# yangye1098/Speech-Denoising-Diffusion-Model-2

Measured on AMD Instinct MI355X. Metric: denoised audio sec/sec, 1000-step UNetModified2 @16kHz, higher is better.
Workload: dtype bf16; 1 GPU; UNetModified2 config_unet.json, linear 1e-6..1e-3, T=1000, 16x16448-sample chunks per GPU, condition_in; model=UNetModified2, global_batch=16, seq_len=16448, parallelism=dp1, lane_rows=16

## Files before the change

### include/sddm_hip.h

```cpp
#ifndef SDDM_HIP_H
#define SDDM_HIP_H
#include <stdint.h>

#ifdef __cplusplus
extern "C" {
#endif

#define SDDM_ABI_VERSION 1

enum sddm_status {
  SDDM_OK = 0,
  SDDM_ERR_NOT_IMPLEMENTED = 1,
  SDDM_ERR_INVALID_ARG = 2,
  SDDM_ERR_SHAPE = 3,
  SDDM_ERR_HIP = 4,
  SDDM_ERR_STATE = 5
};

enum sddm_dtype { SDDM_F32 = 0, SDDM_BF16 = 1, SDDM_F16 = 2 };

enum sddm_transition {
  SDDM_TR_ORIGINAL = 0,
  SDDM_TR_SR3 = 1,
  SDDM_TR_SUPPORTIVE = 2,
  SDDM_TR_CONDITIONAL = 3
};

typedef struct sddm_ctx sddm_ctx;

int sddm_abi_version(void);
const char* sddm_last_error(void);

int sddm_create(int device, int compute_dtype, sddm_ctx** out);
void sddm_destroy(sddm_ctx* ctx);

int sddm_configure(sddm_ctx* ctx, const char* json);

int sddm_load_param(sddm_ctx* ctx, const char* key, const void* host_ptr, const int64_t* shape,
                    int ndim, int src_dtype);

int sddm_missing_params(sddm_ctx* ctx, int64_t* n_missing);

int sddm_sample(sddm_ctx* ctx, const float* cond, int64_t B, int64_t N, uint64_t seed,
                int64_t row_offset, float* out, void* stream);

int sddm_sample_noise(sddm_ctx* ctx, const float* cond, int64_t B, int64_t N, const float* noise, float* out,
                      void* stream);

int sddm_sample_continuous(sddm_ctx* ctx, const float* cond, int64_t B, int64_t N, uint64_t seed,
                           int64_t row_offset, float* out, float* record, int sample_inter, void* stream);

int sddm_network_forward(sddm_ctx* ctx, const float* cond, const float* x_t,
                         const float* noise_level, int64_t B, int64_t N, float* eps_out,
                         void* stream);

int sddm_transition(sddm_ctx* ctx, int mode, const float* x_t, const float* eps,
                    const float* cond, int t, int64_t B, int64_t N, uint64_t seed,
                    int64_t row_offset, float* out, void* stream);

int sddm_q_sample(sddm_ctx* ctx, int mode, const float* x0, const float* y, const float* noise,
                  const int64_t* t, const float* r, int64_t B, int64_t N, float* x_t,
                  float* combined, float* s_out, float* level_out, void* stream);

int sddm_set_conv_tuning(sddm_ctx* ctx, const char* json);

int sddm_log_spectrogram(const float* audio, int64_t B, int64_t N, int n_fft, int hop,
                         const float* window, const float* fb, int n_out, float* out, void* stream);

int sddm_initial_state(sddm_ctx* ctx, int mode, const float* cond, int64_t B, int64_t N,
                       uint64_t seed, int64_t row_offset, float* out, void* stream);

int sddm_schedule(const char* schedule, int n_timestep, double linear_start, double linear_end,
                  float* out);

int sddm_profile_enable(sddm_ctx* ctx, int enable);
int sddm_profile_read(sddm_ctx* ctx, const char* kernel_class, double* avg_ms, int64_t* launches,
                      double* bytes_per_launch, double* flops_per_launch);
int sddm_profile_ops(sddm_ctx* ctx, char* buf, int64_t buflen);

#ifdef __cplusplus
}
#endif
#endif
```

### speech-denoising-diffusion-model-2_amd/csrc/conv_strip_impl.h

```cpp
#pragma once
#include <type_traits>

#ifndef SDDM_ABL_STRIP
#define SDDM_ABL_STRIP 0
#endif
#ifndef SDDM_STRIP_WLD
#define SDDM_STRIP_WLD 1
#endif
#ifndef SDDM_STRIP_WREG
#define SDDM_STRIP_WREG 1
#endif

#include "conv_common.h"
#include "conv_tile_cfg.h"
#include "kernels.h"

namespace sddm {

static constexpr ConvShape kStripShapes[] = {
    {-1, 0, 1, 1, 1, 1, 0, 0, 0, 0, 0, 0, 0, 0, 0, 0, 0},
    {32, 0, 16, 128, 256, 128, 32, 0, 32, 0, 0, 0, 1, 0, 256, 16, 0},
    {32, 0, 16, 128, 256, 128, 32, 0, 32, 0, 0, 1, 1, 0, 256, 16, 0},
    {64, 0, 8, 64, 128, 64, 32, 0, 64, 0, 0, 0, 1, 0, 256, 8, 0},
    {32, 0, 16, 64, 128, 64, 64, 0, 64, 32, 0, 2, 1, 0, 256, 16, 0},
    {32, 0, 16, 64, 128, 64, 64, 0, 64, 0, 0, 0, 0, 1, 256, 16, 0},
    {32, 0, 8, 64, 128, 64, 32, 0, 32, 64, 64, 2, 1, 0, 256, 8, 0},
    {32, 0, 8, 64, 128, 64, 32, 32, 32, 0, 0, 0, 1, 0, 256, 8, 0},
    {32, 0, 8, 64, 128, 64, 32, 0, 32, 32, 32, 2, 1, 0, 256, 8, 0},
    {32, 0, 16, 128, 256, 128, 32, 0, 32, 0, 0, 0, 0, 1, 256, 16, 0},
    {32, 0, 16, 128, 256, 128, 32, 32, 32, 0, 0, 0, 1, 0, 256, 16, 0},
    {32, 0, 16, 128, 256, 128, 32, 0, 32, 32, 32, 2, 1, 0, 256, 16, 0},
    {32, 0, 64, 128, 512, 128, 32, 0, 32, 0, 0, 0, 1, 0, 256, 64, 1},
    {32, 0, 64, 128, 512, 128, 32, 0, 32, 0, 0, 1, 1, 0, 256, 64, 1},
    {64, 0, 64, 64, 256, 64, 32, 0, 64, 0, 0, 0, 1, 0, 256, 64, 1},
    {32, 0, 128, 64, 256, 64, 64, 0, 64, 32, 0, 2, 1, 0, 256, 128, 1},
    {32, 0, 128, 64, 256, 64, 64, 0, 64, 0, 0, 0, 0, 1, 256, 128, 1},
    {32, 0, 64, 64, 256, 64, 32, 0, 32, 64, 64, 2, 1, 0, 256, 64, 1},
    {32, 0, 64, 64, 256, 64, 32, 32, 32, 0, 0, 0, 1, 0, 256, 64, 1},
    {32, 0, 64, 64, 256, 64, 32, 0, 32, 32, 32, 2, 1, 0, 256, 64, 1},
    {32, 0, 64, 128, 512, 128, 32, 0, 32, 0, 0, 0, 0, 1, 256, 64, 1},
    {32, 0, 64, 128, 512, 128, 32, 32, 32, 0, 0, 0, 1, 0, 256, 64, 1},
    {32, 0, 64, 128, 512, 128, 32, 0, 32, 32, 32, 2, 1, 0, 256, 64, 1},
};
static constexpr int kNStripShapes = (int)(sizeof(kStripShapes) / sizeof(kStripShapes[0]));

__host__ inline bool strip_shape_matches(const ConvShape& c, int nblk, int mpi, int SR, const ConvArgs& a) {
  return c.cfg == nblk && c.nw == mpi && c.nb == SR && c.Ho == a.Ho && c.Wo == a.Wo && c.CA == a.CA && c.CB == a.CB &&
         c.Cout == a.Cout && c.RCA == a.RCA && c.RCB == a.RCB && c.res == a.res_mode &&
         c.gn == (a.gamma != nullptr ? 1 : 0) && c.up == (a.upsample ? 1 : 0) && a.n_tiles == c.Ho / SR &&
         a.Hi == (c.up ? c.Ho / 2 : c.Ho) && a.Wi == (c.up ? c.Wo / 2 : c.Wo);
}

template <typename T, int FC, int W, int CIN, int MPI, int RES, bool GN, int SH>
__global__ __launch_bounds__(MPI * 2) void conv_strip_kernel(ConvArgs a, int SR_) {
  constexpr ConvShape SC = kStripShapes[SH];
  constexpr bool CS = SH > 0;
  SDDM_SHAPE_GEO(SC, CS, false, a)
  const int SR = CS ? SC.nb : SR_;
  (void)gTR; (void)gTW; (void)gTX; (void)gRes; (void)gGN; (void)gWo;
  constexpr int NT = MPI * 2;
  constexpr int NWV = NT / 64;
  constexpr int ES = (int)sizeof(T);
  constexpr int NBLK = 16 * FC, FP = 2;
  constexpr int TR = MPI / W, R = 2 * TR + 2;
  constexpr int UPP = CIN * ES / 16;
  constexpr int UPL = ES / 2;
  constexpr int VE = 16 / ES;
  constexpr int PL = ((W + 2) * 16 + 255) / 256 * 256;
  constexpr int SLOT = UPP * PL;
  constexpr int NCK = CIN / 32;
  constexpr int WPL = NBLK * 16;
  constexpr int WPLANES = NCK * 9 * 4 * UPL;
  constexpr int PB = 64 / UPP;
  constexpr int NU = TR * W * UPP;
  constexpr int UPT = NU / NT;
  constexpr int IU = ((TR + 2) * W * UPP + NT - 1) / NT;
  constexpr int RCKM = 4;
  static_assert(UPP >= 1 && UPP <= 64 && (64 % UPP) == 0, "channel units must divide a wave");
  static_assert(NU % NT == 0, "prefetch must split evenly");
  typedef T vec4 __attribute__((ext_vector_type(4)));
  extern __shared__ __attribute__((aligned(16))) char smem[];

  const int tid = threadIdx.x, lane = tid & 63, wave = tid >> 6, g = lane >> 4;
  int strip, b, zb;
  xcd_block<SDDM_XCD_ZIN != 0>(gNT, gCout / NBLK, strip, b, zb);
  const int n0 = zb * NBLK;
  const int H = gHo;
  const int RC = gRCA + gRCB;
  const int rck = RES == 2 ? RC / 32 : 0;
  constexpr bool gn = GN;

  char* ring = smem;
  char* wl = ring + R * SLOT;
  char* rw = wl + WPLANES * WPL;
  const int RPLANES = rck * 32 * ES / 16;
  float* gsc = (float*)(rw + RPLANES * WPL);
  float* red = gsc + 2 * CIN;

  const int y0 = strip * SR;
  const int iters = SR / TR;
  SDDM_STAMP(a, 0);
  GNLoad gl;
  const GNFuse gf{a.gstA, a.gtilesA, a.gntileA, a.gstB, a.gtilesB, a.gntileB, a.gamma, a.beta, a.groups, a.eps};
  gl.issue(gf, b, gCA, gCB, gn, a.bias);
  const T* srcAb = (const T*)a.srcA + (size_t)b * gHi * gWi * gCA;
  const T* srcBb = gCB ? (const T*)a.srcB + (size_t)b * gHi * gWi * gCB : srcAb;
  f32x4 ini[IU];
#pragma unroll
  for (int k = 0; k < IU; ++k) {
    const int u = min(tid + k * NT, (TR + 2) * W * UPP - 1);
    const int grp = u >> 6, j = u & 63;
    const int pix = grp * PB + (j % PB), q = j / PB, r = pix / W, x = pix % W;
    const int ry = min(max(y0 - 1 + r, 0), H - 1);
    const int sy = gUp ? ry >> 1 : ry, sx = gUp ? x >> 1 : x;
    const int c0 = q * VE;
    const bool fa = c0 < gCA;
    ini[k] = *(const f32x4*)((fa ? srcAb : srcBb) + ((size_t)sy * gWi + sx) * (fa ? gCA : gCB) + (fa ? c0 : c0 - gCA));
  }
  constexpr int WUN = NBLK * WPLANES, WU = (WUN + NT - 1) / NT;
  constexpr bool WLD = SDDM_STRIP_WLD && WU <= 12;
  constexpr int RUN_MAX = RES == 2 ? NBLK * RCKM * 4 * UPL : 0, RU = (RUN_MAX + NT - 1) / NT;
  const int RUN = NBLK * RPLANES;
  f32x4 wst[WLD ? WU : 1], rst[WLD && RU > 0 ? RU : 1];
  if constexpr (WLD) {
#pragma unroll
    for (int i = 0; i < WU; ++i) {
      const int u0 = tid + i * NT, u = u0 < WUN ? u0 : 0;
      const int co = u % NBLK, pl = u / NBLK;
      const char* src;
      if constexpr (ES == 2) {
        src = (const char*)a.wgt_t + ((size_t)pl * gCout + n0 + co) * 16;
      } else {
        const int ck = pl / (9 * 4 * UPL), rem = pl - ck * 9 * 4 * UPL, tap = rem / (4 * UPL), un = rem - tap * 4 * UPL;
        src = (const char*)a.wgt + ((((size_t)(n0 + co) * NCK + ck) * 9 + tap) * 32) * ES + un * 16;
      }
      wst[i] = *(const f32x4*)src;
    }
    if constexpr (RES == 2) {
#pragma unroll
      for (int i = 0; i < RU; ++i) {
        const int u0 = tid + i * NT, u = u0 < RUN ? u0 : 0;
        const int co = u % NBLK, pl = u / NBLK;
        const char* src = ES == 2 ? (const char*)a.res_wgt_t + ((size_t)pl * gCout + n0 + co) * 16
                                  : (const char*)a.res_wgt + ((size_t)(n0 + co) * RC) * ES + pl * 16;
        rst[i] = *(const f32x4*)src;
      }
    }
  } else {
    for (int u0 = wave * 64; u0 < NBLK * WPLANES; u0 += NT) {
      const int u = u0 + lane;
      const int co = u % NBLK, pl = u / NBLK;
      const char* src;
      if constexpr (ES == 2) {
        src = (const char*)a.wgt_t + ((size_t)pl * gCout + n0 + co) * 16;
      } else {
        const int ck = pl / (9 * 4 * UPL), rem = pl - ck * 9 * 4 * UPL, tap = rem / (4 * UPL), un = rem - tap * 4 * UPL;
        src = (const char*)a.wgt + ((((size_t)(n0 + co) * NCK + ck) * 9 + tap) * 32) * ES + un * 16;
      }
      __builtin_amdgcn_global_load_lds((const __attribute__((address_space(1))) void*)src,
                                       (__attribute__((address_space(3))) void*)(wl + u0 * 16), 16, 0, 0);
    }
    if constexpr (RES == 2) {
      for (int u0 = wave * 64; u0 < NBLK * RPLANES; u0 += NT) {
        const int u = u0 + lane;
        const int co = u % NBLK, pl = u / NBLK;
        const char* src = ES == 2 ? (const char*)a.res_wgt_t + ((size_t)pl * gCout + n0 + co) * 16
                                  : (const char*)a.res_wgt + ((size_t)(n0 + co) * RC) * ES + pl * 16;
        __builtin_amdgcn_global_load_lds((const __attribute__((address_space(1))) void*)src,
                                         (__attribute__((address_space(3))) void*)(rw + u0 * 16), 16, 0, 0);
      }
    }
  }
  for (int u = tid; u < R * UPP * 2; u += NT) {
    const int side = u & 1, pl = u >> 1;
    *(f32x4*)(ring + pl * PL + (side ? (W + 1) : 0) * 16) = f32x4{0.f, 0.f, 0.f, 0.f};
  }
  if (gn) gl.finish(gf, b, gCA, gCB, gsc, gsc + CIN);
  __syncthreads();
  const int t_now = a.t_dev ? *a.t_dev : 0;
  const float* trow = a.temb ? a.temb + (size_t)(a.temb_per_b ? b : t_now) * a.temb_ld : a.bias;
  float badd[FC][4];
#pragma unroll
  for (int fc = 0; fc < FC; ++fc)
#pragma unroll
    for (int i = 0; i < 4; ++i) {
      const int co = n0 + fc * 16 + 4 * g + i;
      const float bv = a.bias[co], tv = trow[co];
      badd[fc][i] = bv + (a.temb ? tv : 0.f);
    }
  float sshift;
  {
    const int cs = n0 + (tid % NBLK);
    const float bv = a.bias[cs], tv = trow[cs];
    sshift = bv + (a.temb ? tv : 0.f);
  }
  const int base = ((y0 - 1) % R + R) % R;
#pragma unroll
  for (int k = 0; k < IU; ++k) {
    const int u = tid + k * NT;
    if (u >= (TR + 2) * W * UPP) break;
    const int grp = u >> 6, j = u & 63;
    const int pix = grp * PB + (j % PB), q = j / PB, r = pix / W, x = pix % W;
    const int ry = y0 - 1 + r;
    f32x4 v = ini[k];
    if (ry < 0 || ry >= H) v = f32x4{0.f, 0.f, 0.f, 0.f};
    else if (gn) v = transform_fast<T>(v, gsc + q * VE, gsc + CIN + q * VE);
    *(f32x4*)(ring + ((base + r) % R) * SLOT + q * PL + (x + 1) * 16) = v;
  }

  if constexpr (WLD) {
#pragma unroll
    for (int i = 0; i < WU; ++i)
      if (tid + i * NT < WUN) *(f32x4*)(wl + (tid + i * NT) * 16) = wst[i];
    if constexpr (RES == 2) {
#pragma unroll
      for (int i = 0; i < RU; ++i)
        if (tid + i * NT < RUN) *(f32x4*)(rw + (tid + i * NT) * 16) = rst[i];
    }
  }

  static_assert(W % 32 == 0, "a wave's 32 pixels must not cross rows");
  const int wave_u = __builtin_amdgcn_readfirstlane(wave);
  int prow[FP], pcol[FP];
#pragma unroll
  for (int fp = 0; fp < FP; ++fp) {
    prow[fp] = (wave_u * 32) / W;
    pcol[fp] = (wave_u * 32) % W + fp * 16 + (lane & 15);
  }
  int pr[UPT], loff[UPT], cq[UPT];
  const char* rsrc_[UPT];
  unsigned rstr[UPT];
#pragma unroll
  for (int k = 0; k < UPT; ++k) {
    const int u = tid + k * NT, grp = u >> 6, j = u & 63;
    const int pix = grp * PB + (j % PB);
    const int q = j / PB, x = pix % W;
    pr[k] = pix / W;
    loff[k] = q * PL + (x + 1) * 16;
    cq[k] = q * VE;
    const int c0 = q * VE;
    const int sx = gUp ? (x >> 1) : x;
    const bool fa = c0 < gCA;
    rsrc_[k] = fa ? (const char*)(srcAb + sx * gCA + c0) : (const char*)(srcBb + sx * gCB + (c0 - gCA));
    rstr[k] = (unsigned)(gWi * (fa ? gCA : gCB) * ES);
  }
  auto issue_rows = [&](f32x4 (&dst)[UPT], int j) {
#pragma unroll
    for (int k = 0; k < UPT; ++k) {
      const int ry = min(y0 + j * TR + 1 + pr[k], H - 1);
      const int sy = gUp ? (ry >> 1) : ry;
      dst[k] = *(const f32x4*)(rsrc_[k] + (unsigned)__umul24((unsigned)sy, rstr[k]));
    }
  };
  auto xform_unit = [&](const f32x4 (&src)[UPT], int j, int k) {
    const int ry = y0 + j * TR + 1 + pr[k];
    f32x4 v = src[k];
    if constexpr (GN) v = transform_lds<T>(v, gsc + cq[k], gsc + CIN + cq[k]);
    return ry >= H ? f32x4{0.f, 0.f, 0.f, 0.f} : v;
  };
  auto store_rows = [&](const f32x4 (&tv)[UPT], int j) {
    const int sb = (base + j * TR + 2) % R;
#pragma unroll
    for (int k = 0; k < UPT; ++k) {
      int sl = sb + pr[k];
      sl = sl >= R ? sl - R : sl;
      *(f32x4*)(ring + (int)__umul24(sl, SLOT) + loff[k]) = tv[k];
    }
  };
  T* outb = (T*)a.out + (size_t)b * H * W * gCout;
  const T* resb = RES == 1 ? (const T*)a.res_src + (size_t)b * H * W * gCout : outb;
  auto issue_res1 = [&](vec4 (&dst)[FP][FC], int it) {
#pragma unroll
    for (int fp = 0; fp < FP; ++fp) {
      const int yy = min(y0 + it * TR, H - TR) + prow[fp];
      const unsigned po = (unsigned)(yy * W * gCout) + __umul24((unsigned)pcol[fp], (unsigned)gCout) + n0 + 4 * g;
#pragma unroll
      for (int fc = 0; fc < FC; ++fc) dst[fp][fc] = *(const vec4*)((const char*)resb + (po * ES + fc * 16 * ES));
    }
  };
  const T* rawAb = RES == 2 ? (const T*)a.rawA + (size_t)b * H * W * gRCA : outb;
  const T* rawBb = (RES == 2 && gRCB) ? (const T*)a.rawB + (size_t)b * H * W * gRCB : rawAb;
  auto issue_res2 = [&](Frag<T> (&dst)[RCKM][FP], int it) {
#pragma unroll
    for (int ck = 0; ck < RCKM; ++ck)
#pragma unroll
      for (int fp = 0; fp < FP; ++fp) {
        const int yy = min(y0 + it * TR, H - TR) + prow[fp];
        const int c0 = min(ck, rck - 1) * 32 + g * 8;
        const int pix = yy * W + pcol[fp];
        const T* sp = c0 < gRCA ? rawAb + ((int)__umul24(pix, gRCA) + c0) : rawBb + ((int)__umul24(pix, gRCB) + (c0 - gRCA));
        dst[ck][fp] = load_frag<T>((const char*)sp);
      }
  };

  f32x2 s1[FC][2], s2[FC][2], bp[FC][2];
#pragma unroll
  for (int fc = 0; fc < FC; ++fc)
#pragma unroll
    for (int h = 0; h < 2; ++h) {
      s1[fc][h] = f32x2{0.f, 0.f};
      s2[fc][h] = f32x2{0.f, 0.f};
      bp[fc][h] = f32x2{badd[fc][2 * h], badd[fc][2 * h + 1]};
    }
  const char* abase = wl + g * UPL * WPL + (lane & 15) * 16;
  const char* rbase = rw + g * UPL * WPL + (lane & 15) * 16;

  f32x4 rowsA[UPT], rowsB[UPT];
  vec4 r1A[FP][FC], r1B[FP][FC];
  Frag<T> r2A[RCKM][FP], r2B[RCKM][FP];
  constexpr bool WREG = SDDM_STRIP_WREG && ES == 2 && NCK == 1 && FC == 2 && RES != 2 && MPI == 256;
  Frag<T> wreg[WREG ? 9 : 1][FC];
  auto body = [&](auto LR, auto LX, int it, f32x4 (&nxt)[UPT], f32x4 (&fill)[UPT], vec4 (&r1cur)[FP][FC],
                  vec4 (&r1nxt)[FP][FC], Frag<T> (&r2cur)[RCKM][FP], Frag<T> (&r2nxt)[RCKM][FP]) {
    const int y = y0 + it * TR;
    const int s_it = (base + it * TR) % R;
#ifdef SDDM_STAMPS
    const int dbg = a.dbg;
#else
    constexpr int dbg = 0;
#endif
    if constexpr (decltype(LR)::value) if (!(dbg & 4)) issue_rows(nxt, it + 2);
    if constexpr (RES == 1 && decltype(LX)::value) if (!(dbg & 64)) issue_res1(r1nxt, it + 1);
    if constexpr (RES == 2 && decltype(LX)::value) issue_res2(r2nxt, it + 1);
    __builtin_amdgcn_sched_barrier(0);
    f32x4 acc[FP][FC];
#pragma unroll
    for (int i = 0; i < FP; ++i)
#pragma unroll
      for (int j = 0; j < FC; ++j) acc[i][j] = f32x4{0.f, 0.f, 0.f, 0.f};
    const char* bptr[FP][3];
#pragma unroll
    for (int fp = 0; fp < FP; ++fp)
#pragma unroll
      for (int dy = 0; dy < 3; ++dy) {
        int sl = s_it + prow[fp] + dy;
        sl = sl >= R ? sl - R : sl;
        bptr[fp][dy] = ring + (sl * SLOT + (g * UPL * PL + pcol[fp] * 16));
      }
    f32x4 tv[UPT];
#pragma unroll
    for (int ck = 0; ck < NCK; ++ck) {
#pragma unroll
      for (int tap = 0; tap < 9; ++tap) {
        const int dy = tap / 3, dx = tap - 3 * dy;
        Frag<T> bf[FP];
#pragma unroll
        for (int fp = 0; fp < FP; ++fp)
          bf[fp] = load_planes<T>((SDDM_ABL_STRIP & 256) ? bptr[fp][0] : bptr[fp][dy] + ck * 4 * UPL * PL + dx * 16, PL);
#pragma unroll
        for (int fc = 0; fc < FC; ++fc) {
          const Frag<T> af = WREG ? wreg[WREG ? tap : 0][fc]
                                  : load_planes<T>(abase + ((SDDM_ABL_STRIP & 16) ? 0 : (ck * 9 + tap) * 4 * UPL * WPL) + fc * 256, WPL);
#pragma unroll
          for (int fp = 0; fp < FP; ++fp)
            if (!(dbg & 8)) mfma_frag(acc[fp][fc], af, bf[fp]);
        }
#pragma unroll
        for (int k = 0; k < UPT; ++k)
          if (decltype(LX)::value && ck * 9 + tap == k * 9 * NCK / UPT) tv[k] = (dbg & 2) ? fill[k] : xform_unit(fill, it + 1, k);
      }
    }
    if constexpr (RES == 2) {
#pragma unroll
      for (int ck = 0; ck < RCKM; ++ck) {
        if (ck >= rck) break;
#pragma unroll
        for (int fc = 0; fc < FC; ++fc) {
          const Frag<T> af = load_planes<T>(rbase + ck * 4 * UPL * WPL + fc * 256, WPL);
#pragma unroll
          for (int fp = 0; fp < FP; ++fp) mfma_frag(acc[fp][fc], af, r2cur[ck][fp]);
        }
      }
    }
#pragma unroll
    for (int fp = 0; fp < FP; ++fp) {
      const unsigned po = (unsigned)((y + prow[fp]) * W * gCout) + __umul24((unsigned)pcol[fp], (unsigned)gCout);
#pragma unroll
      for (int fc = 0; fc < FC; ++fc) {
        const unsigned co = n0 + fc * 16 + 4 * g;
        f32x2 d0 = f32x2{acc[fp][fc][0], acc[fp][fc][1]}, d1 = f32x2{acc[fp][fc][2], acc[fp][fc][3]};
        if constexpr (RES == 1) {
          d0 += unpack2<T>(r1cur[fp][fc][0], r1cur[fp][fc][1]);
          d1 += unpack2<T>(r1cur[fp][fc][2], r1cur[fp][fc][3]);
        }
        if (!(dbg & 128)) store4p<T>((T*)((char*)outb + (po + co) * ES), d0 + bp[fc][0], d1 + bp[fc][1]);
        s1[fc][0] += d0;
        s1[fc][1] += d1;
        s2[fc][0] = __builtin_elementwise_fma(d0, d0, s2[fc][0]);
        s2[fc][1] = __builtin_elementwise_fma(d1, d1, s2[fc][1]);
      }
    }
    if constexpr (decltype(LX)::value) store_rows(tv, it + 1);
    lds_sync();
  };
  issue_rows(rowsA, 1);
  if constexpr (RES == 1) issue_res1(r1A, 0);
  if constexpr (RES == 2) issue_res2(r2A, 0);
  constexpr int NYOUNG = UPT + (RES == 1 ? FP * FC : 0) + (RES == 2 ? RCKM * FP : 0);
  static_assert(NYOUNG < 64, "vmcnt is a 6-bit counter");
  asm volatile("s_waitcnt vmcnt(%0) lgkmcnt(0)\n\ts_barrier" :: "n"(NYOUNG) : "memory");
  if constexpr (WREG) {
#pragma unroll
    for (int tap = 0; tap < 9; ++tap)
#pragma unroll
      for (int fc = 0; fc < FC; ++fc) wreg[tap][fc] = load_planes<T>(abase + tap * 4 * UPL * WPL + fc * 256, WPL);
  }
  SDDM_STAMP(a, 3);
  using yes = std::integral_constant<bool, true>;
  using no = std::integral_constant<bool, false>;
  for (int it = 0; it < iters - 2; it += 2) {
    body(yes{}, yes{}, it, rowsB, rowsA, r1A, r1B, r2A, r2B);
    body(yes{}, yes{}, it + 1, rowsA, rowsB, r1B, r1A, r2B, r2A);
  }
  body(no{}, yes{}, iters - 2, rowsB, rowsA, r1A, r1B, r2A, r2B);
  body(no{}, no{}, iters - 1, rowsA, rowsB, r1B, r1A, r2B, r2A);

  SDDM_STAMP(a, 4);
  if (a.stats) {
    const float nl = (float)(FP * iters) * 16.f;
#pragma unroll
    for (int fc = 0; fc < FC; ++fc)
#pragma unroll
      for (int i = 0; i < 4; ++i) {
        const float t1 = row_sum16(s1[fc][i >> 1][i & 1]), t2 = row_sum16(s2[fc][i >> 1][i & 1]);
        if ((lane & 15) == 0) {
          float* rr = red + ((wave * NBLK) + fc * 16 + 4 * g + i) * 3;
          rr[0] = nl; rr[1] = t1; rr[2] = t2;
        }
      }
    lds_sync();
    if (tid < NBLK) {
      float n = 0.f, u1 = 0.f, u2 = 0.f;
      for (int w = 0; w < NWV; ++w) {
        const float* rr = red + (w * NBLK + tid) * 3;
        n += rr[0]; u1 += rr[1]; u2 += rr[2];
      }
      float* dst = a.stats + (((size_t)b * gNT + strip) * gCout + n0 + tid) * 2;
      dst[0] = (sshift + u1 / n) * n;
      dst[1] = fmaxf(u2 - u1 * u1 / n, 0.f);
    }
  }
  SDDM_STAMP(a, 6);
  SDDM_STAMP(a, 7);
}

template <typename T, int FC, int W, int CIN, int MPI>
static size_t strip_lds(const ConvArgs& a) {
  constexpr int ES = (int)sizeof(T), NBLK = 16 * FC, TR = MPI / W, R = 2 * TR + 2;
  constexpr int UPP = CIN * ES / 16, PL = ((W + 2) * 16 + 255) / 256 * 256;
  size_t n = (size_t)R * UPP * PL + (size_t)(CIN / 32) * 9 * 4 * (ES / 2) * NBLK * 16;
  if (a.res_mode == 2) n += (size_t)((a.RCA + a.RCB) * ES / 16) * NBLK * 16;
  n += (size_t)2 * CIN * 4 + (size_t)(MPI / 32) * NBLK * 3 * 4;
  return n;
}

template <typename T, int FC, int W, int CIN, int MPI, int SH = 0>
static hipError_t strip_go(const ConvArgs& a, int SR, int B, hipStream_t s, size_t* lo) {
  const size_t lds = strip_lds<T, FC, W, CIN, MPI>(a);
  if (lo) { *lo = lds; return hipSuccess; }
  constexpr int TR = MPI / W;
  if (lds > kLdsBytes || a.Ho % SR || SR % (2 * TR) || a.Cout % (16 * FC) || a.res_mode < 0 || a.res_mode > 2 ||
      (a.res_mode == 2 && (a.RCA + a.RCB) > 128))
    return hipErrorInvalidValue;
  if (a.n_tiles != a.Ho / SR) return hipErrorInvalidValue;
  if (sizeof(T) == 2 && (!a.wgt_t || (a.res_mode == 2 && !a.res_wgt_t))) return hipErrorInvalidValue;
  const dim3 grid = xcd_grid(a.Ho / SR, B, a.Cout / (16 * FC)), blk(MPI * 2);
  if (a.res_mode != 0 && !a.gamma) return hipErrorInvalidValue;
  if constexpr (SH > 0) {
    constexpr ConvShape c = kStripShapes[SH];
    hipLaunchKernelGGL((conv_strip_kernel<T, FC, W, CIN, MPI, c.res, c.gn != 0, SH>), grid, blk, lds, s, a, SR);
  } else if (a.res_mode == 0 && !a.gamma) hipLaunchKernelGGL((conv_strip_kernel<T, FC, W, CIN, MPI, 0, false, 0>), grid, blk, lds, s, a, SR);
  else if (a.res_mode == 0) hipLaunchKernelGGL((conv_strip_kernel<T, FC, W, CIN, MPI, 0, true, 0>), grid, blk, lds, s, a, SR);
  else if (a.res_mode == 1) hipLaunchKernelGGL((conv_strip_kernel<T, FC, W, CIN, MPI, 1, true, 0>), grid, blk, lds, s, a, SR);
  else hipLaunchKernelGGL((conv_strip_kernel<T, FC, W, CIN, MPI, 2, true, 0>), grid, blk, lds, s, a, SR);
  return hipGetLastError();
}

template <typename T, int SH>
static bool strip_shape_go(const ConvArgs& a, int nblk, int mpi, int SR, int B, hipStream_t s, hipError_t& e) {
  if constexpr (SH >= kNStripShapes || sizeof(T) == 4) {
    return false;
  } else if constexpr (!shape_for_type<T>(kStripShapes[SH])) {
    return strip_shape_go<T, SH + 1>(a, nblk, mpi, SR, B, s, e);
  } else {
    constexpr ConvShape c = kStripShapes[SH];
    if (strip_shape_matches(c, nblk, mpi, SR, a)) {
      e = strip_go<T, c.cfg / 16, c.Wo, c.CA + c.CB, c.nw, SH>(a, SR, B, s, nullptr);
      return true;
    }
    return strip_shape_go<T, SH + 1>(a, nblk, mpi, SR, B, s, e);
  }
}

template <typename T>
hipError_t strip_dispatch(const ConvArgs& a, int nblk, int mpi, int SR, int B, hipStream_t s, size_t* lo) {
  static const bool generic = std::getenv("SDDM_NO_STRIP_SHAPES") != nullptr;
  hipError_t e;
  if (!lo && !generic && strip_shape_go<T, 1>(a, nblk, mpi, SR, B, s, e)) return e;
  const int Cin = a.CA + a.CB;
#define SDDM_STRIP(FCV, WV, CV)                                                                   \
  if (nblk == 16 * FCV && a.Wo == WV && Cin == CV)                                                \
    return mpi == 256 ? strip_go<T, FCV, WV, CV, 256>(a, SR, B, s, lo) : strip_go<T, FCV, WV, CV, 128>(a, SR, B, s, lo);
  SDDM_STRIP(2, 128, 32) SDDM_STRIP(2, 128, 64) SDDM_STRIP(4, 128, 32) SDDM_STRIP(4, 128, 64)
  SDDM_STRIP(2, 64, 32) SDDM_STRIP(2, 64, 64) SDDM_STRIP(2, 64, 128)
  SDDM_STRIP(4, 64, 32) SDDM_STRIP(4, 64, 64) SDDM_STRIP(4, 64, 128)
#undef SDDM_STRIP
  if (lo) *lo = (size_t)1 << 40;
  return hipErrorInvalidValue;
}

}
```

### speech-denoising-diffusion-model-2_amd/csrc/sddm_runtime.cpp

```cpp
#include <hip/hip_runtime.h>

#include <algorithm>
#include <cstdarg>
#include <cstdlib>
#include <cstdio>
#include <cstring>
#include <functional>
#include <map>
#include <set>
#include <memory>
#include <string>
#include <vector>

#include "../../include/sddm_hip.h"
#include "json_mini.h"
#include "kernels.h"
#include "q_kernels.h"
#include "stft_kernels.h"
#include "sddm_common.h"

namespace sddm {
int compute_schedule(const std::string& schedule, int T, double linear_start, double linear_end,
                     float* out);
}
using namespace sddm;

static thread_local std::string g_last_error;
static void sddm_set_error(int code, const char* fmt, ...) {
  char buf[1024];
  va_list ap;
  va_start(ap, fmt);
  vsnprintf(buf, sizeof(buf), fmt, ap);
  va_end(ap);
  g_last_error = buf;
  (void)code;
}
#define FAIL(code, ...)                 \
  do {                                  \
    sddm_set_error(code, __VA_ARGS__);  \
    return code;                        \
  } while (0)

static const char* kTableNames[14] = {"betas", "alphas", "alpha_bar", "sqrt_alpha_bar",
                                      "predicted_noise_coeff", "sigma", "supportive_gamma",
                                      "supportive_sigma_hat", "m", "sqrt_delta", "c_xt", "c_yt",
                                      "c_epst", "sqrt_delta_estimated"};

static uint16_t f32_to_bf16_bits(float f) {
  uint32_t u;
  std::memcpy(&u, &f, 4);
  if ((u & 0x7f800000u) == 0x7f800000u && (u & 0x7fffffu)) return (uint16_t)((u >> 16) | 0x40);
  u += 0x7fffu + ((u >> 16) & 1u);
  return (uint16_t)(u >> 16);
}
static uint16_t f32_to_f16_bits(float f) {
  _Float16 h = (_Float16)f;
  uint16_t r;
  std::memcpy(&r, &h, 2);
  return r;
}
static size_t dtype_size(int dt) { return dt == DT_F32 ? 4 : 2; }
static const char* dt_name(int dt) { return dt == DT_F32 ? "f32" : dt == DT_BF16 ? "bf16" : "f16"; }
static void store_elem(void* base, size_t idx, float v, int dt) {
  if (dt == DT_F32) ((float*)base)[idx] = v;
  else if (dt == DT_BF16) ((uint16_t*)base)[idx] = f32_to_bf16_bits(v);
  else ((uint16_t*)base)[idx] = f32_to_f16_bits(v);
}

struct Arena {
  char* base = nullptr;
  size_t cap = 0, used = 0;
  std::vector<std::pair<size_t, size_t>> pending;
  size_t reserve(size_t bytes) {
    const size_t off = (used + 255) & ~(size_t)255;
    used = off + bytes;
    return off;
  }
  hipError_t commit() {
    if (base) { (void)hipFree(base); base = nullptr; }
    cap = used;
    if (cap == 0) return hipSuccess;
    hipError_t e = hipMalloc(&base, cap);
    if (e == hipSuccess) e = hipMemset(base, 0, cap);
    return e;
  }
  void reset() {
    if (base) (void)hipFree(base);
    base = nullptr; cap = used = 0;
  }
  template <typename T> T* at(size_t off) const { return (T*)(base + off); }
};

struct UNetCfg {
  int in_channel = 2, out_channel = 1, inner = 32, groups = 32, res_blocks = 3;
  std::vector<int> mults{1, 2, 3, 4, 5};
  int seg = 128, stride = 64;
  double dropout = 0.0;
};
struct LayerDesc { int kind; std::string name; int cin, cout; };
static std::vector<LayerDesc> unet_layers(const UNetCfg& c, std::vector<LayerDesc>* downs_out,
                                          std::vector<LayerDesc>* mid_out, std::vector<LayerDesc>* ups_out) {
  std::vector<LayerDesc> downs, mid, ups;
  downs.push_back({0, "downs.0", c.in_channel, c.inner});
  std::vector<int> feat{c.inner};
  int cin = c.inner, idx = 1, cout = c.inner;
  for (size_t ind = 0; ind < c.mults.size(); ++ind) {
    cout = c.inner * c.mults[ind];
    for (int r = 0; r < c.res_blocks; ++r) {
      downs.push_back({1, "downs." + std::to_string(idx++), cin, cout});
      feat.push_back(cout);
      cin = cout;
    }
    downs.push_back({2, "downs." + std::to_string(idx++), cout, cout});
    feat.push_back(cout);
  }
  mid.push_back({1, "mid.0", cin, cin});
  idx = 0;
  for (int ind = (int)c.mults.size() - 1; ind >= 0; --ind) {
    cin = c.inner * c.mults[ind];
    cout = cin;
    ups.push_back({1, "ups." + std::to_string(idx++), cin + feat.back(), cout});
    feat.pop_back();
    ups.push_back({3, "ups." + std::to_string(idx++), cout, cout});
    cout = ind == 0 ? c.inner : c.inner * c.mults[ind - 1];
    for (int r = 0; r < c.res_blocks; ++r) {
      ups.push_back({1, "ups." + std::to_string(idx++), cin + feat.back(), cout});
      feat.pop_back();
      cin = cout;
    }
  }
  std::vector<LayerDesc> all;
  all.insert(all.end(), downs.begin(), downs.end());
  all.insert(all.end(), mid.begin(), mid.end());
  all.insert(all.end(), ups.begin(), ups.end());
  all.push_back({4, "final_conv", cout, c.out_channel});
  if (downs_out) *downs_out = downs;
  if (mid_out) *mid_out = mid;
  if (ups_out) *ups_out = ups;
  return all;
}

static std::map<std::string, std::vector<int64_t>> unet_param_shapes(const UNetCfg& c) {
  std::map<std::string, std::vector<int64_t>> s;
  const int64_t inner = c.inner;
  s["noise_level_mlp.1.weight"] = {inner * 4, inner};
  s["noise_level_mlp.1.bias"] = {inner * 4};
  s["noise_level_mlp.3.weight"] = {inner, inner * 4};
  s["noise_level_mlp.3.bias"] = {inner};
  for (const auto& L : unet_layers(c, nullptr, nullptr, nullptr)) {
    const std::string& n = L.name;
    if (L.kind == 1) {
      s[n + ".noise_func.noise_func.0.weight"] = {L.cout, inner};
      s[n + ".noise_func.noise_func.0.bias"] = {L.cout};
      s[n + ".block1.block.0.weight"] = {L.cin};
      s[n + ".block1.block.0.bias"] = {L.cin};
      s[n + ".block1.block.3.weight"] = {L.cout, L.cin, 3, 3};
      s[n + ".block1.block.3.bias"] = {L.cout};
      s[n + ".block2.block.0.weight"] = {L.cout};
      s[n + ".block2.block.0.bias"] = {L.cout};
      s[n + ".block2.block.3.weight"] = {L.cout, L.cout, 3, 3};
      s[n + ".block2.block.3.bias"] = {L.cout};
      if (L.cin != L.cout) {
        s[n + ".res_conv.weight"] = {L.cout, L.cin, 1, 1};
        s[n + ".res_conv.bias"] = {L.cout};
      }
    } else if (L.kind == 2 || L.kind == 3) {
      s[n + ".conv.weight"] = {L.cout, L.cin, 3, 3};
      s[n + ".conv.bias"] = {L.cout};
    } else if (L.kind == 0) {
      s[n + ".weight"] = {L.cout, L.cin, 3, 3};
      s[n + ".bias"] = {L.cout};
    } else {
      s[n + ".block.0.weight"] = {L.cin};
      s[n + ".block.0.bias"] = {L.cin};
      s[n + ".block.3.weight"] = {L.cout, L.cin, 3, 3};
      s[n + ".block.3.bias"] = {L.cout};
    }
  }
  return s;
}

struct Param { std::vector<int64_t> shape; std::vector<float> data; bool loaded = false; };
struct Tensor { void* p = nullptr; int C = 0, H = 0, W = 0; float* stats = nullptr; int tiles = 0, n_tile = 0; };
struct Op {
  int cls;
  double bytes, flops;
  std::function<hipError_t(hipStream_t)> run;
  std::string name = "";
  std::function<hipError_t(hipStream_t, int)> run_dbg = nullptr;
  std::string kname = "";
  std::string kinst = "";
};
struct ProfAcc { double ms = 0; int64_t n = 0; double bytes = 0, flops = 0; };

struct RunState {
  const float* cond = nullptr;
  float* x = nullptr;
  const float* temb = nullptr;
  int temb_per_b = 0;
  int* t_dev = nullptr;
  int final_mode = 0;
  float* eps_out = nullptr;
  uint64_t seed = 0;
  int64_t row_offset = 0;
  const float* noise = nullptr;
  int64_t noise_ld = 0;
};

static constexpr int kStreams = 4;
static constexpr int kMaxLanes = 64;

struct Lane {
  int B = 0, row0 = 0, idx = 0;
  Arena arena;
  std::vector<Op> ops;
  RunState rs;
  size_t off_temb_fwd = 0, off_cond = 0, off_x = 0;
  hipGraphExec_t gexec = nullptr;
  hipGraph_t graph = nullptr;
  int g_K = 0, g_gen = -1;
  ~Lane() {
    if (gexec) (void)hipGraphExecDestroy(gexec);
    if (graph) (void)hipGraphDestroy(graph);
    arena.reset();
  }
};

struct DWState;
struct WGState;
struct WUState;

struct sddm_ctx {
  int device = 0, dtype = DT_BF16;
  bool configured = false;
  std::string arch_type, net_type, p_transition = "original";
  int noise_time_step = 0;
  int tr_mode = SDDM_TR_ORIGINAL, init_mode = 0;
  int T = 0, num_samples = -1;
  std::vector<float> tables;
  bool tables_dirty = true;
  UNetCfg ucfg;
  std::map<std::string, Param> params;
  bool params_dirty = true;
  Arena warena;
  size_t off_tables = 0, off_tdev = 0, off_temb_tab = 0;
  std::map<std::string, size_t> woff;
  int SC = 0;
  std::map<std::string, int> temb_off;
  std::vector<std::unique_ptr<Lane>> lanes;
  int plan_B = -1;
  int lane_rows = 16;
  int plan_gen = 0;
  hipStream_t work[kStreams] = {};
  hipEvent_t ev_in = nullptr;
  hipEvent_t ev_done[kStreams] = {};
  bool use_graphs = true;
  unsigned long long* stamp_buf = nullptr;
  int64_t stamp_blocks = 0;
  bool prof = false;
  std::vector<hipEvent_t> ev_pool;
  std::vector<std::pair<int, int>> ev_pend;
  std::vector<ProfAcc> op_acc;
  std::shared_ptr<DWState> dws;
  std::shared_ptr<WGState> wgs;
  std::shared_ptr<WUState> wus;
  struct KernTune { int kind, a, b, c; };
  struct TuneTable {
    std::map<std::string, std::pair<int, int>> deep_tune;
    std::map<std::string, KernTune> kern_tune;
    int B = -1, dtype = -1, N = -1;
  };
  std::vector<TuneTable> tunes;
  int hop_samples = 256;

  const float* dtab(int k) const { return warena.at<float>(off_tables) + (size_t)k * (T + 1); }
  TransCoef coef() const {
    TransCoef c;
    c.betas = dtab(0); c.alphas = dtab(1); c.sqrt_alpha_bar = dtab(3); c.pnc = dtab(4);
    c.sigma = dtab(5); c.sgamma = dtab(6); c.ssh = dtab(7); c.sqrt_delta = dtab(9);
    c.c_xt = dtab(10); c.c_yt = dtab(11); c.c_epst = dtab(12); c.sde = dtab(13);
    return c;
  }
};

static int upload_weights(sddm_ctx* c) {
  const int dt = c->dtype;
  const size_t es = dtype_size(dt);
  auto P = [&](const std::string& k) -> const Param& { return c->params.at(k); };
  c->warena.reset();
  c->woff.clear();
  c->temb_off.clear();
  Arena& A = c->warena;
  struct Blob { size_t off; std::vector<char> bytes; };
  std::vector<Blob> blobs;
  auto add_f32 = [&](const std::string& name, const std::vector<float>& v) {
    Blob b;
    b.bytes.resize(v.size() * 4);
    std::memcpy(b.bytes.data(), v.data(), b.bytes.size());
    b.off = A.reserve(b.bytes.size());
    c->woff[name] = b.off;
    blobs.push_back(std::move(b));
  };
  auto add_conv3 = [&](const std::string& name, const Param& w) {
    const int co = (int)w.shape[0], ci = (int)w.shape[1];
    const int cop = (co + 63) / 64 * 64, nch = ci / 32;
    Blob b;
    b.bytes.assign((size_t)cop * ci * 9 * es, 0);
    for (int o = 0; o < co; ++o)
      for (int i = 0; i < ci; ++i)
        for (int tap = 0; tap < 9; ++tap) {
          const size_t dst = (((size_t)o * nch + i / 32) * 9 + tap) * 32 + (i % 32);
          store_elem(b.bytes.data(), dst, w.data[((size_t)o * ci + i) * 9 + tap], dt);
        }
    b.off = A.reserve(b.bytes.size());
    c->woff[name] = b.off;
    blobs.push_back(std::move(b));
    {
      Blob bf;
      const int ns = (ci / 32) * 9;
      bf.bytes.assign((size_t)co * ci * 9 * es, 0);
      for (int o = 0; o < co; ++o)
        for (int i = 0; i < ci; ++i)
          for (int tap = 0; tap < 9; ++tap) {
            const int s = (i / 32) * 9 + tap, l = (o % 16) + 16 * ((i % 32) / 8);
            const size_t dst = (((size_t)(o / 16) * ns + s) * 64 + l) * 8 + i % 8;
            store_elem(bf.bytes.data(), dst, w.data[((size_t)o * ci + i) * 9 + tap], dt);
          }
      bf.off = A.reserve(bf.bytes.size());
      c->woff[name + "_f"] = bf.off;
      blobs.push_back(std::move(bf));
    }
    if (dt != DT_F32) {
      Blob bt;
      bt.bytes.assign((size_t)co * ci * 9 * es, 0);
      for (int o = 0; o < co; ++o)
        for (int i = 0; i < ci; ++i)
          for (int tap = 0; tap < 9; ++tap) {
            const size_t dst = ((((size_t)(i / 32) * 9 + tap) * 4 + (i % 32) / 8) * co + o) * 8 + i % 8;
            store_elem(bt.bytes.data(), dst, w.data[((size_t)o * ci + i) * 9 + tap], dt);
          }
      bt.off = A.reserve(bt.bytes.size());
      c->woff[name + "_t"] = bt.off;
      blobs.push_back(std::move(bt));
    }
  };
  auto add_conv1 = [&](const std::string& name, const Param& w) {
    const int co = (int)w.shape[0], ci = (int)w.shape[1];
    const int cop = (co + 63) / 64 * 64;
    Blob b;
    b.bytes.assign((size_t)cop * ci * es, 0);
    for (int o = 0; o < co; ++o)
      for (int i = 0; i < ci; ++i) store_elem(b.bytes.data(), (size_t)o * ci + i, w.data[(size_t)o * ci + i], dt);
    b.off = A.reserve(b.bytes.size());
    c->woff[name] = b.off;
    blobs.push_back(std::move(b));
    {
      Blob bf;
      bf.bytes.assign((size_t)co * ci * es, 0);
      for (int o = 0; o < co; ++o)
        for (int i = 0; i < ci; ++i) {
          const int l = (o % 16) + 16 * ((i % 32) / 8);
          store_elem(bf.bytes.data(), (((size_t)(o / 16) * (ci / 32) + i / 32) * 64 + l) * 8 + i % 8,
                     w.data[(size_t)o * ci + i], dt);
        }
      bf.off = A.reserve(bf.bytes.size());
      c->woff[name + "_f"] = bf.off;
      blobs.push_back(std::move(bf));
    }
    if (dt != DT_F32) {
      Blob bt;
      bt.bytes.assign((size_t)co * ci * es, 0);
      for (int o = 0; o < co; ++o)
        for (int i = 0; i < ci; ++i)
          store_elem(bt.bytes.data(), (((size_t)(i / 32) * 4 + (i % 32) / 8) * co + o) * 8 + i % 8,
                     w.data[(size_t)o * ci + i], dt);
      bt.off = A.reserve(bt.bytes.size());
      c->woff[name + "_t"] = bt.off;
      blobs.push_back(std::move(bt));
    }
  };
  const std::string pfx = "";
  std::vector<float> pw, pb;
  int sc = 0;
  for (const auto& L : unet_layers(c->ucfg, nullptr, nullptr, nullptr)) {
    const std::string& n = L.name;
    if (L.kind == 0) {
      add_f32(n + ".weight", P(n + ".weight").data);
      add_f32(n + ".bias", P(n + ".bias").data);
    } else if (L.kind == 1) {
      add_f32(n + ".block1.gamma", P(n + ".block1.block.0.weight").data);
      add_f32(n + ".block1.beta", P(n + ".block1.block.0.bias").data);
      add_conv3(n + ".block1.w", P(n + ".block1.block.3.weight"));
      add_f32(n + ".block1.b", P(n + ".block1.block.3.bias").data);
      add_f32(n + ".block2.gamma", P(n + ".block2.block.0.weight").data);
      add_f32(n + ".block2.beta", P(n + ".block2.block.0.bias").data);
      add_conv3(n + ".block2.w", P(n + ".block2.block.3.weight"));
      std::vector<float> b2 = P(n + ".block2.block.3.bias").data;
      if (L.cin != L.cout) {
        add_conv1(n + ".res.w", P(n + ".res_conv.weight"));
        const auto& rb = P(n + ".res_conv.bias").data;
        for (int i = 0; i < L.cout; ++i) b2[i] = b2[i] + rb[i];
      }
      add_f32(n + ".block2.b", b2);
      const auto& fw = P(n + ".noise_func.noise_func.0.weight").data;
      const auto& fb = P(n + ".noise_func.noise_func.0.bias").data;
      pw.insert(pw.end(), fw.begin(), fw.end());
      pb.insert(pb.end(), fb.begin(), fb.end());
      c->temb_off[n] = sc;
      sc += L.cout;
    } else if (L.kind == 2 || L.kind == 3) {
      add_conv3(n + ".w", P(n + ".conv.weight"));
      add_f32(n + ".b", P(n + ".conv.bias").data);
    } else {
      add_f32(n + ".gamma", P(n + ".block.0.weight").data);
      add_f32(n + ".beta", P(n + ".block.0.bias").data);
      add_f32(n + ".w", P(n + ".block.3.weight").data);
      add_f32(n + ".b", P(n + ".block.3.bias").data);
    }
  }
  add_f32("mlp.w1", P("noise_level_mlp.1.weight").data);
  add_f32("mlp.b1", P("noise_level_mlp.1.bias").data);
  add_f32("mlp.w2", P("noise_level_mlp.3.weight").data);
  add_f32("mlp.b2", P("noise_level_mlp.3.bias").data);
  add_f32("proj.w", pw);
  add_f32("proj.b", pb);
  {
    const int half = c->ucfg.inner / 2;
    std::vector<float> ev(half);
    for (int k = 0; k < half; ++k) {
      const float e = (-(float)k * 4.0f) / (float)half;
      ev[k] = 1e4f * std::pow(10.0f, e);
    }
    add_f32("emb_vec", ev);
  }
  c->SC = sc;
  c->off_tables = A.reserve(sizeof(float) * 14 * (c->T + 1));
  c->off_tdev = A.reserve(64 * kMaxLanes);
  c->off_temb_tab = A.reserve(sizeof(float) * (size_t)(c->T + 1) * sc);
  SDDM_HIP_CHECK(A.commit());
  for (const auto& b : blobs) SDDM_HIP_CHECK(hipMemcpy(A.base + b.off, b.bytes.data(), b.bytes.size(), hipMemcpyHostToDevice));
  c->params_dirty = false;
  c->tables_dirty = true;
  c->plan_B = -1;
  return SDDM_OK;
}

static int upload_tables(sddm_ctx* c) {
  SDDM_HIP_CHECK(hipMemcpy(c->warena.base + c->off_tables, c->tables.data(), sizeof(float) * c->tables.size(),
                           hipMemcpyHostToDevice));
  c->tables_dirty = false;
  return SDDM_OK;
}

#include "dw_runtime.h"
#include "wg_runtime.h"
#include "wu_runtime.h"

struct ConvChoice {
  int strip = 0;
  int nblk = 32, SR = 0, mpi = 128;
  int mt = 0, ckb = 0, nw = 4, nb = 32;
  int tile = -1;
  int TR = 0, TW = 0, tiles_x = 0, n_tiles = 0;
  int chain = 0;
};

static bool choose_deep(int dt, int B, ConvArgs a, bool s2, ConvChoice& ch, int want_mt = 0, int want_nw = 0,
                        int want_nb = 0) {
  static int force_mt = -1, force_nw = -1, force_nb = 0;
  if (force_mt < 0) {
    force_mt = force_nw = 0;
    if (const char* e = std::getenv("SDDM_DEEP_CFG")) std::sscanf(e, "%d:%d:%d", &force_mt, &force_nw, &force_nb);
  }
  const int nb = want_mt ? (want_nb ? want_nb : 32) : (force_nb && a.Cout % force_nb == 0 ? force_nb : 32);
  if (a.Cout % nb) return false;
  const int nz = a.Cout / nb;
  a.deep_nb = nb;
  struct Cand { int mt, nw, TR, TW, tiles_x, n_tiles, blocks, rounds; };
  std::vector<Cand> cs;
  for (int mt : {128, 64, 32, 16}) {
    if (mt == 16 && nb != 16) continue;
    const int TW = std::min(a.Wo, mt);
    if (mt % TW || a.Wo % TW) continue;
    const int TR = std::min(mt / TW, a.Ho);
    if (a.Ho % TR) continue;
    if (TR * TW < mt && mt > 32) continue;
    a.TR = TR; a.TW = TW; a.tiles_x = a.Wo / TW; a.n_tiles = a.tiles_x * (a.Ho / TR);
    for (int nw : {8, 4}) {
      a.deep_nw = nw;
      if (conv_deep_lds_bytes(dt, mt, s2, a) > kLdsBytes) continue;
      const int blocks = a.n_tiles * B * nz, per_round = 256 * (nw == 4 ? 2 : 1);
      cs.push_back({mt, nw, TR, TW, a.tiles_x, a.n_tiles, blocks, (blocks + per_round - 1) / per_round});
    }
  }
  if (cs.empty()) return false;
  const Cand* pick = nullptr;
  const int fm = want_mt ? want_mt : force_mt, fn = want_mt ? want_nw : force_nw;
  for (const Cand& c : cs)
    if (c.mt == fm && c.nw == fn) pick = &c;
  if (!pick) {
    pick = &cs[0];
    for (const Cand& c : cs) {
      if (c.rounds != pick->rounds) { if (c.rounds < pick->rounds) pick = &c; continue; }
      if (c.nw != pick->nw) { if (c.nw > pick->nw) pick = &c; continue; }
      if (c.mt < pick->mt) pick = &c;
    }
  }
  ch.strip = 0; ch.mt = pick->mt; ch.nw = pick->nw; ch.nb = nb; ch.ckb = (a.CA + a.CB) / 32;
  ch.TR = pick->TR; ch.TW = pick->TW; ch.tiles_x = pick->tiles_x; ch.n_tiles = pick->n_tiles;
  return true;
}

static int deep_zin(const ConvArgs& a, int B, size_t es) {
  static const int force = std::getenv("SDDM_DEEP_ZIN") ? std::atoi(std::getenv("SDDM_DEEP_ZIN")) : -1;
  if (force >= 0) return force;
  const double in = (double)B * a.Hi * a.Wi * (a.CA + a.CB) * es;
  const double w = (double)a.Cout * ((a.CA + a.CB) * 9 + (a.res_mode == 2 ? a.RCA + a.RCB : 0)) * es;
  return in >= w ? 1 : 0;
}

static bool choose_tile(int dt, int B, ConvArgs a, bool s2, ConvChoice& ch, int want = -1) {
  if (dt == DT_F32) return false;
  static const int force = std::getenv("SDDM_TILE_CFG") ? std::atoi(std::getenv("SDDM_TILE_CFG")) : -1;
  static const bool off = std::getenv("SDDM_NO_TILE") != nullptr;
  if (off) return false;
  const int fw = want >= 0 ? want : force;
  struct Cand { int cfg, TR, TW, tiles_x, n_tiles, blocks, area; };
  std::vector<Cand> cs;
  for (int cfg = 0; cfg < conv_tile_ncfg(); ++cfg) {
    const TileCfg t = conv_tile_cfg(cfg);
    const int MT = t.wpx * t.fp * 16, NB = t.wco * t.fc * 16;
    if (a.Cout % NB) continue;
    const int TW = std::min(a.Wo, MT);
    if (MT % TW || a.Wo % TW) continue;
    const int TR = std::min(MT / TW, a.Ho);
    if (a.Ho % TR) continue;
    if (TR * TW < MT && (TR != a.Ho || TW != a.Wo)) continue;
    a.TR = TR; a.TW = TW; a.tiles_x = a.Wo / TW; a.n_tiles = a.tiles_x * (a.Ho / TR);
    if (conv_tile_lds_bytes(cfg, s2, a) > kLdsBytes) continue;
    cs.push_back({cfg, TR, TW, a.tiles_x, a.n_tiles, a.n_tiles * B * (a.Cout / NB), TR * TW * NB});
  }
  if (cs.empty()) return false;
  const Cand* pick = nullptr;
  for (const Cand& c : cs)
    if (c.cfg == fw) pick = &c;
  if (!pick) {
    for (const Cand& c : cs) {
      if (!pick) { pick = &c; continue; }
      const bool cf = c.blocks >= 256, pf = pick->blocks >= 256;
      if (cf != pf) { if (cf) pick = &c; continue; }
      if (!cf) { if (c.blocks != pick->blocks) { if (c.blocks > pick->blocks) pick = &c; continue; } }
      if (c.area > pick->area) pick = &c;
    }
  }
  ch.strip = 0; ch.tile = pick->cfg;
  ch.TR = pick->TR; ch.TW = pick->TW; ch.tiles_x = pick->tiles_x; ch.n_tiles = pick->n_tiles;
  return true;
}

static bool choose_conv(int dt, int B, int Cin, int RC, int res_mode, int Ho, int Wo, int Cout, bool s2, bool up,
                        ConvChoice& ch, int want_mt = 0, int want_nw = 0, int kind = 0, int ka = 0, int want_nb = 0) {
  ConvArgs a{};
  a.CA = Cin; a.CB = 0; a.RCA = RC; a.RCB = 0; a.res_mode = res_mode; a.Ho = Ho; a.Wo = Wo; a.Cout = Cout;
  a.upsample = up ? 1 : 0;
  a.Hi = up ? Ho / 2 : (s2 ? Ho * 2 : Ho); a.Wi = up ? Wo / 2 : (s2 ? Wo * 2 : Wo);
  static const int env_mpi = std::getenv("SDDM_STRIP_MPI") ? std::atoi(std::getenv("SDDM_STRIP_MPI")) : 0;
  static const int env_blocks = std::getenv("SDDM_STRIP_BLOCKS") ? std::atoi(std::getenv("SDDM_STRIP_BLOCKS")) : 0;
  if (kind == 2) {
    ConvChoice t = ch;
    if (choose_tile(dt, B, a, s2, t, ka) && t.tile == ka) { ch = t; return true; }
  }
  if (!s2 && (Wo == 128 || Wo == 64) && std::getenv("SDDM_NO_STRIP") == nullptr && (kind == 0 || kind == 1)) {
    const int nbs[2] = {(Cout % 64 == 0) ? 64 : 32, 32};
    for (int mpi : {256, 128}) {
      if (env_mpi && mpi != env_mpi) continue;
      const int TRs = mpi / Wo;
      if (Ho % TRs) continue;
      for (int ni = 0; ni < 2; ++ni) {
        const int nb = nbs[ni];
        if (conv_strip_lds_bytes(dt, nb, mpi, a) > kLdsBytes) continue;
        const int nz = (Cout + nb - 1) / nb;
        int SR = 0;
        const int target = env_blocks ? env_blocks : 256;
        for (int m = 32; m >= 2; m /= 2) {
          const int sr = TRs * m;
          if (Ho % sr) continue;
          SR = sr;
          if ((Ho / sr) * B * nz >= target) break;
        }
        if (SR == 0) continue;
        ch.strip = 1; ch.nblk = nb; ch.SR = SR; ch.mpi = mpi;
        ch.TR = SR; ch.TW = Wo; ch.tiles_x = 1; ch.n_tiles = Ho / SR;
        return true;
      }
    }
  }
  if (want_mt == 0 && kind != 3 && choose_tile(dt, B, a, s2, ch)) return true;
  return choose_deep(dt, B, a, s2, ch, want_mt, want_nw, want_nb);
}

static int build_lane(sddm_ctx* c, Lane& L) {
  const int B = L.B;
  Lane* lp = &L;
  const int dt = c->dtype;
  const size_t es = dtype_size(dt);
  const UNetCfg& u = c->ucfg;
  const int N = c->num_samples, W = u.seg, S = u.stride;
  const int F = (N - W) / S + 1;
  L.ops.clear();
  L.arena.reset();
  Arena& A = L.arena;

  struct TRes { size_t p, st; int C, H, W, tiles, n_tile; };
  std::vector<TRes> tres;
  auto new_tensor = [&](int C, int H, int Wd, int tiles, int n_tile) -> int {
    TRes t;
    t.p = A.reserve((size_t)B * H * Wd * C * es);
    t.st = A.reserve(sizeof(float) * (size_t)B * tiles * C * 2);
    t.C = C; t.H = H; t.W = Wd; t.tiles = tiles; t.n_tile = n_tile;
    tres.push_back(t);
    return (int)tres.size() - 1;
  };
  struct GNRes { int a, b; std::string w; };
  std::vector<GNRes> gres;
  auto new_gn = [&](int xa, int xb, const std::string& w) -> int {
    gres.push_back({xa, xb, w});
    return (int)gres.size() - 1;
  };
  L.off_temb_fwd = A.reserve(sizeof(float) * (size_t)B * std::max(c->SC, 1));
  L.off_cond = A.reserve(sizeof(float) * (size_t)B * N);
  L.off_x = A.reserve(sizeof(float) * (size_t)B * N);

  enum { ST_CONVIN, ST_GN, ST_CONV, ST_FINAL };
  struct Step {
    int type = 0;
    std::string w;
    std::string rb;
    int srcA = -1, srcB = -1, gn = -1, out = -1;
    int s2 = 0, up = 0, res_mode = 0, rawA = -1, rawB = -1, cout = 0;
    bool temb = false;
    ConvChoice ch;
  };
  std::vector<Step> prog;
  const int PB = std::max(1, c->lane_rows);
  const sddm_ctx::TuneTable* tuned = nullptr;
  for (const auto& tt : c->tunes)
    if (tt.B == PB && tt.N == N && tt.dtype == dt) { tuned = &tt; break; }
  if (!tuned && dt == DT_F16)
    for (const auto& tt : c->tunes)
      if (tt.B == PB && tt.N == N && tt.dtype == DT_BF16) { tuned = &tt; break; }
  auto pick = [&](const std::string& name, int Cin, int RC, int res_mode, int Ho, int Wo, int cout, bool s2, bool up,
                  ConvChoice& ch) {
    int wm = 0, wn = 0, wb = 0, kind = 0, ka = 0;
    if (tuned) {
      auto it = tuned->deep_tune.find(name);
      if (it != tuned->deep_tune.end()) { wm = it->second.first; wn = it->second.second; kind = 3; }
      auto kt = tuned->kern_tune.find(name);
      if (kt != tuned->kern_tune.end()) {
        kind = kt->second.kind; ka = kt->second.a;
        if (kind == 3) { wm = kt->second.a; wn = kt->second.b; wb = kt->second.c; }
      }
    }
    const bool chain = kind == 4 && dt != DT_F32;
    if (kind == 4) kind = 0;
    const bool ok = choose_conv(dt, PB, Cin, RC, res_mode, Ho, Wo, cout, s2, up, ch, wm, wn, kind, ka, wb);
    ch.chain = chain ? 1 : 0;
    return ok;
  };
  const int TRin = 512 / W;
  if (u.inner != 32 || 512 % W || F % TRin || (TRin + 1) * S + W + 2 > 1024)
    FAIL(SDDM_ERR_NOT_IMPLEMENTED, "conv_in needs inner_channel 32 and segment_len dividing 512 (got %d, %d)", u.inner, W);
  const int t0 = new_tensor(u.inner, F, W, F / TRin, TRin * W);
  { Step st; st.type = ST_CONVIN; st.out = t0; prog.push_back(st); }

  auto res_block = [&](const std::string& n, int xa, int xb, int cin, int cout) -> int {
    const int H = tres[xa].H, Wd = tres[xa].W;
    ConvChoice c1, c2;
    if (!pick(n + ".block1", cin, 0, 0, H, Wd, cout, false, false, c1)) return -1;
    if (!pick(n + ".block2", cout, cin, cin != cout ? 2 : 1, H, Wd, cout, false, false, c2)) return -1;
    const int g1 = new_gn(xa, xb, n + ".block1");
    const int h = new_tensor(cout, H, Wd, c1.n_tiles, c1.TR * c1.TW);
    { Step st; st.type = ST_CONV; st.w = n + ".block1"; st.rb = n; st.srcA = xa; st.srcB = xb; st.gn = g1;
      st.out = h; st.cout = cout; st.temb = true; st.ch = c1; prog.push_back(st); }
    const int g2 = new_gn(h, -1, n + ".block2");
    const int o = new_tensor(cout, H, Wd, c2.n_tiles, c2.TR * c2.TW);
    { Step st; st.type = ST_CONV; st.w = n + ".block2"; st.rb = n; st.srcA = h; st.gn = g2; st.out = o;
      st.cout = cout; st.res_mode = cin != cout ? 2 : 1; st.rawA = xa; st.rawB = xb; st.ch = c2; prog.push_back(st); }
    return o;
  };
  std::vector<LayerDesc> downs, mid, ups;
  unet_layers(u, &downs, &mid, &ups);
  std::vector<int> feats{t0};
  int cur = t0;
  for (size_t i = 1; i < downs.size(); ++i) {
    const LayerDesc& L = downs[i];
    if (L.kind == 1) {
      cur = res_block(L.name, cur, -1, L.cin, L.cout);
    } else {
      if (tres[cur].H % 2 || tres[cur].W % 2) FAIL(SDDM_ERR_SHAPE, "odd size before %s", L.name.c_str());
      const int H = tres[cur].H / 2, Wd = tres[cur].W / 2;
      ConvChoice ch;
      if (!pick(L.name, tres[cur].C, 0, 0, H, Wd, L.cout, true, false, ch)) FAIL(SDDM_ERR_SHAPE, "no tile for %s", L.name.c_str());
      const int o = new_tensor(L.cout, H, Wd, ch.n_tiles, ch.TR * ch.TW);
      Step st; st.type = ST_CONV; st.w = L.name; st.srcA = cur; st.out = o; st.s2 = 1; st.cout = L.cout; st.ch = ch;
      prog.push_back(st);
      cur = o;
    }
    if (cur < 0) FAIL(SDDM_ERR_SHAPE, "no tile for %s", L.name.c_str());
    feats.push_back(cur);
  }
  for (const LayerDesc& L : mid) {
    cur = res_block(L.name, cur, -1, L.cin, L.cout);
    if (cur < 0) FAIL(SDDM_ERR_SHAPE, "no tile for %s", L.name.c_str());
  }
  for (const LayerDesc& L : ups) {
    if (L.kind == 1) {
      const int skip = feats.back();
      feats.pop_back();
      if (tres[skip].H != tres[cur].H || tres[skip].W != tres[cur].W)
        FAIL(SDDM_ERR_SHAPE, "skip/upsample size mismatch at %s (torch.cat would raise)", L.name.c_str());
      cur = res_block(L.name, cur, skip, L.cin, L.cout);
      if (cur < 0) FAIL(SDDM_ERR_SHAPE, "no tile for %s", L.name.c_str());
    } else {
      const int H = tres[cur].H * 2, Wd = tres[cur].W * 2;
      ConvChoice ch;
      if (!pick(L.name, tres[cur].C, 0, 0, H, Wd, L.cout, false, true, ch)) FAIL(SDDM_ERR_SHAPE, "no tile for %s", L.name.c_str());
      const int o = new_tensor(L.cout, H, Wd, ch.n_tiles, ch.TR * ch.TW);
      Step st; st.type = ST_CONV; st.w = L.name; st.srcA = cur; st.out = o; st.up = 1; st.cout = L.cout; st.ch = ch;
      prog.push_back(st);
      cur = o;
    }
  }
  const int gf = new_gn(cur, -1, "final_conv");
  { Step st; st.type = ST_FINAL; st.srcA = cur; st.gn = gf; prog.push_back(st); }

  SDDM_HIP_CHECK(A.commit());

  auto TT = [&](int i) {
    Tensor t;
    if (i < 0) return t;
    const TRes& r = tres[i];
    t.p = A.base + r.p; t.stats = A.at<float>(r.st); t.C = r.C; t.H = r.H; t.W = r.W;
    t.tiles = r.tiles; t.n_tile = r.n_tile;
    return t;
  };
  auto WF = [&](const std::string& k) { return c->warena.at<float>(c->woff.at(k)); };
  auto WV = [&](const std::string& k) { return (const void*)(c->warena.base + c->woff.at(k)); };
  auto conv_args = [&](const Step& st, ConvArgs& a, double& bytes, double& flops) -> int {
    a = ConvArgs{};
    const Tensor sa = TT(st.srcA), sb = TT(st.srcB), o = TT(st.out);
    a.srcA = sa.p; a.srcB = sb.p; a.CA = sa.C; a.CB = sb.C;
    a.Hi = sa.H; a.Wi = sa.W; a.Ho = o.H; a.Wo = o.W; a.upsample = st.up;
    a.Cout = st.cout; a.out = o.p; a.stats = o.stats;
    if (st.gn >= 0) {
      const GNRes& gr = gres[st.gn];
      const Tensor ga = TT(gr.a), gb = TT(gr.b);
      a.gstA = ga.stats; a.gtilesA = ga.tiles; a.gntileA = ga.n_tile;
      a.gstB = gb.stats; a.gtilesB = gb.tiles; a.gntileB = gb.n_tile;
      a.gamma = WF(gr.w + ".gamma"); a.beta = WF(gr.w + ".beta"); a.groups = u.groups; a.eps = 1e-5f;
      const int Ct = ga.C + gb.C;
      if (Ct % u.groups || (gb.C && ga.C % (Ct / u.groups)) || 256 % u.groups)
        FAIL(SDDM_ERR_SHAPE, "GroupNorm(%d, %d) at %s: unsupported grouping", u.groups, Ct, gr.w.c_str());
    }
    a.wgt = WV(st.w + ".w"); a.bias = WF(st.w + ".b");
    a.wgt_t = c->woff.count(st.w + ".w_t") ? WV(st.w + ".w_t") : nullptr;
    a.wgt_f = WV(st.w + ".w_f");
    a.res_mode = st.res_mode;
    const int Cin = a.CA + a.CB;
    bytes = (double)B * a.Hi * a.Wi * Cin * es + (double)B * a.Ho * a.Wo * a.Cout * es +
            (double)a.Cout * 9 * Cin * es;
    flops = 2.0 * B * a.Ho * a.Wo * a.Cout * 9.0 * Cin;
    if (st.res_mode == 1) {
      a.res_src = TT(st.rawA).p;
      bytes += (double)B * a.Ho * a.Wo * a.Cout * es;
    } else if (st.res_mode == 2) {
      const Tensor ra = TT(st.rawA), rb = TT(st.rawB);
      a.rawA = ra.p; a.rawB = rb.p; a.RCA = ra.C; a.RCB = rb.C;
      a.res_wgt = WV(st.rb + ".res.w");
      a.res_wgt_t = c->woff.count(st.rb + ".res.w_t") ? WV(st.rb + ".res.w_t") : nullptr;
      a.res_wgt_f = WV(st.rb + ".res.w_f");
      if ((ra.C + rb.C) % 32) FAIL(SDDM_ERR_SHAPE, "%s.res_conv: channels must be multiples of 32", st.rb.c_str());
      bytes += (double)B * a.Ho * a.Wo * (ra.C + rb.C) * es + (double)a.Cout * (ra.C + rb.C) * es;
      flops += 2.0 * B * a.Ho * a.Wo * a.Cout * (double)(ra.C + rb.C);
    }
    const ConvChoice& ch = st.ch;
    a.TR = ch.TR; a.TW = ch.TW; a.tiles_x = ch.tiles_x; a.n_tiles = ch.n_tiles;
    if (a.n_tiles != o.tiles || a.TR * a.TW != o.n_tile) FAIL(SDDM_ERR_STATE, "tile mismatch for %s", st.w.c_str());
    if ((a.CA + a.CB) % 32 || a.Cout % 32) FAIL(SDDM_ERR_SHAPE, "%s: channels must be multiples of 32", st.w.c_str());
    return SDDM_OK;
  };
  sddm_ctx* ctx = c;
  for (size_t si = 0; si < prog.size(); ++si) {
    const Step& st = prog[si];
    if (st.type == ST_CONV && st.ch.chain) {
      if (si + 4 >= prog.size()) FAIL(SDDM_ERR_SHAPE, "chain: %s is not followed by mid.0 / ups.0", st.w.c_str());
      const Step* S5[5] = {&prog[si], &prog[si + 1], &prog[si + 2], &prog[si + 3], &prog[si + 4]};
      const char* want[5] = {nullptr, "mid.0.block1", "mid.0.block2", "ups.0.block1", "ups.0.block2"};
      for (int k = 0; k < 5; ++k)
        if (S5[k]->type != ST_CONV || !S5[k]->ch.chain || (k > 0 && S5[k]->w != want[k]) || (k == 0 && !S5[k]->s2))
          FAIL(SDDM_ERR_SHAPE, "chain: the tuning table must mark the last Downsample, mid.0.block1/2 and ups.0.block1/2 (got %s)",
               S5[k]->w.c_str());
      ConvArgs ca[5];
      double bytes = 0, flops = 0;
      for (int k = 0; k < 5; ++k) {
        double by = 0, fl = 0;
        if (const int r = conv_args(*S5[k], ca[k], by, fl)) return r;
        flops += fl;
      }
      const int Cc = ca[0].Cout, Hc = ca[0].Ho, Wc = ca[0].Wo;
      if (ca[1].CA != Cc || ca[3].CA != Cc || ca[3].CB != Cc || ca[4].res_mode != 2 || ca[4].RCA != Cc || ca[4].RCB != Cc ||
          ca[2].res_mode != 1 || ca[3].srcB != ca[0].out || ca[4].rawB != ca[0].out)
        FAIL(SDDM_ERR_SHAPE, "chain: unexpected bottom-level wiring");
      ChainArgs x{};
      x.x = ca[0].srcA; x.out = ca[4].out;
      for (int k = 0; k < 5; ++k) { x.wgt[k] = ca[k].wgt_f; x.bias[k] = ca[k].bias; }
      for (int k = 0; k < 4; ++k) { x.gamma[k] = ca[k + 1].gamma; x.beta[k] = ca[k + 1].beta; }
      x.res_wgt = ca[4].res_wgt_f;
      x.temb_ld = c->SC; x.C = Cc; x.H = Hc; x.W = Wc; x.groups = u.groups; x.eps = 1e-5f;
      bytes = (double)B * (2 * Hc) * (2 * Wc) * Cc * es + (double)B * Hc * Wc * Cc * es;
      for (int k = 0; k < 5; ++k) bytes += (double)ca[k].Cout * (ca[k].CA + ca[k].CB) * 9 * es;
      bytes += (double)Cc * 2 * Cc * es;
      const int toff_m = c->temb_off.at("mid.0"), toff_u = c->temb_off.at("ups.0");
      std::string nm;
      for (int k = 0; k < 5; ++k) nm += (k ? "+" : "") + S5[k]->w;
      L.ops.push_back({2, bytes, flops, [lp, x, dt, B, toff_m, toff_u](hipStream_t s) {
                          ChainArgs y = x;
                          y.temb[0] = lp->rs.temb ? lp->rs.temb + toff_m : nullptr;
                          y.temb[1] = lp->rs.temb ? lp->rs.temb + toff_u : nullptr;
                          y.temb_per_b = lp->rs.temb_per_b;
                          y.t_dev = lp->rs.t_dev;
                          return launch_conv_chain(dt, y, B, s);
                        }, nm + "[chain]"});
      char kn[96];
      snprintf(kn, sizeof(kn), "conv_chain_kernel<%s,%d,%d,%d>", dt_name(dt), Cc, Hc, Wc);
      L.ops.back().kname = kn;
      L.ops.back().kinst = kn;
      si += 4;
      continue;
    }
    if (st.type == ST_CONVIN) {
      ConvInArgs a{};
      a.N = N; a.F = F; a.W = W; a.S = S; a.Cout = u.inner;
      a.w = WF("downs.0.weight"); a.bias = WF("downs.0.bias");
      const Tensor o = TT(st.out);
      a.out = o.p; a.stats = o.stats; a.TR = TRin;
      const double bytes = (double)B * N * 4 * 2 + (double)B * F * W * u.inner * es;
      const double flops = 2.0 * B * F * W * u.inner * 18;
#ifdef SDDM_STAMPS
      if (const char* sn = std::getenv("SDDM_STAMPS"))
        if (std::string(sn) == "downs.0") {
          if (!c->stamp_buf) SDDM_HIP_CHECK(hipMalloc(&c->stamp_buf, sizeof(unsigned long long) * 8 * 65536));
          a.stamps = c->stamp_buf;
          c->stamp_blocks = (int64_t)(F / TRin) * B;
        }
#endif
      L.ops.push_back({0, bytes, flops, [lp, a, dt, B](hipStream_t s) {
                          ConvInArgs x = a;
                          x.cond = lp->rs.cond; x.x = lp->rs.x; x.t_dev = lp->rs.t_dev;
                          return launch_conv_in(dt, x, B, s);
                        }, "downs.0"});
      L.ops.back().kname = std::string("conv_in_kernel<") + dt_name(dt) + ">";
      L.ops.back().kinst = L.ops.back().kname;
    } else if (st.type == ST_CONV) {
      ConvArgs a;
      double bytes = 0, flops = 0;
      if (const int r = conv_args(st, a, bytes, flops)) return r;
      const int Cin = a.CA + a.CB;
      const ConvChoice ch = st.ch;
      const bool s2 = st.s2 != 0;
      const bool temb = st.temb;
      if (std::getenv("SDDM_PRINT_SHAPES"))
        fprintf(stderr, "SHAPE %s %s%d s2=%d TR=%d TW=%d Ho=%d Wo=%d CA=%d CB=%d Cout=%d RCA=%d RCB=%d res=%d gn=%d up=%d mt=%d nw=%d nb=%d nblk=%d mpi=%d SR=%d ntiles=%d\n",
                st.w.c_str(), ch.strip ? "strip" : (ch.tile >= 0 ? "tile" : "deep"), ch.tile >= 0 ? ch.tile : ch.mt, s2 ? 1 : 0,
                a.TR, a.TW, a.Ho, a.Wo, a.CA, a.CB, a.Cout, a.RCA, a.RCB, a.res_mode, a.gamma ? 1 : 0, a.upsample ? 1 : 0,
                ch.mt, ch.nw, ch.nb, ch.nblk, ch.mpi, ch.SR, a.n_tiles);
      const int toff = temb ? c->temb_off.at(st.rb) : 0;
#ifdef SDDM_STAMPS
      if (const char* sn = std::getenv("SDDM_STAMPS")) {
        if (st.w == sn) {
          if (!c->stamp_buf) SDDM_HIP_CHECK(hipMalloc(&c->stamp_buf, sizeof(unsigned long long) * 8 * 65536));
          SDDM_HIP_CHECK(hipMemset(c->stamp_buf, 0, sizeof(unsigned long long) * 8 * 65536));
          a.stamps = c->stamp_buf;
          if (const char* f = std::getenv("SDDM_STAMPS_DBG")) a.dbg = std::atoi(f);
          int nb = 32;
          if (ch.tile >= 0) { const TileCfg tc = conv_tile_cfg(ch.tile); nb = tc.wco * tc.fc * 16; }
          c->stamp_blocks = ch.strip ? (int64_t)(a.Ho / ch.SR) * B * ((a.Cout + ch.nblk - 1) / ch.nblk)
                                     : (int64_t)a.n_tiles * B * (a.Cout / (ch.tile >= 0 ? nb : ch.nb));
        }
      }
#endif
      L.ops.push_back({2, bytes, flops, [ctx, lp, a, s2, ch, dt, B, temb, toff](hipStream_t s) {
                          ConvArgs x = a;
                          if (temb) {
                            x.temb = lp->rs.temb + toff;
                            x.temb_ld = ctx->SC;
                            x.temb_per_b = lp->rs.temb_per_b;
                            x.t_dev = lp->rs.t_dev;
                          }
                          if (ch.strip) return launch_conv_strip(dt, ch.nblk, ch.mpi, ch.SR, x, B, s);
                          if (ch.tile >= 0) return launch_conv_tile(dt, ch.tile, s2, x, B, s);
                          x.deep_zin = deep_zin(x, B, dtype_size(dt)); x.deep_nw = ch.nw; x.deep_nb = ch.nb;
                          return launch_conv_deep(dt, ch.mt, s2, x, B, s);
                        }, st.w + (ch.strip ? "[strip]" : (ch.tile >= 0 ? "[tile" + std::to_string(ch.tile) + "]"
                                                                         : "[deep" + std::to_string(ch.mt) + "_" + std::to_string(ch.nw) + "_" + std::to_string(ch.nb) + "]"))});
      {
        char kn[160];
        if (ch.strip)
          snprintf(kn, sizeof(kn), "conv_strip_kernel<%s,%d,%d,%d,%d>", dt_name(dt), ch.nblk / 16, a.Wo, Cin, ch.mpi);
        else if (ch.tile >= 0) {
          const TileCfg tc = conv_tile_cfg(ch.tile);
          snprintf(kn, sizeof(kn), "conv_tile_kernel<%s,%d,%d,%d,%d,%d> (tile%d)", dt_name(dt), s2 ? 1 : 0, tc.wpx, tc.wco,
                   tc.fp, tc.fc, ch.tile);
        } else
          snprintf(kn, sizeof(kn), "conv_deep_kernel<%s,%d,%d,%d,%d>", dt_name(dt), s2 ? 1 : 0, ch.mt, ch.nw, ch.nb);
        L.ops.back().kname = kn;
        char ki[192];
        if (ch.strip)
          snprintf(ki, sizeof(ki), "conv_strip_kernel<%s,%d,%d,%d,%d,%d,%d>", dt_name(dt), ch.nblk / 16, a.Wo, Cin,
                   ch.mpi, a.res_mode, a.gamma ? 1 : 0);
        else if (ch.tile >= 0)
          snprintf(ki, sizeof(ki), "%s", kn);
        else
          snprintf(ki, sizeof(ki), "conv_deep_kernel<%s,%d,%d,%d,%d,%d>", dt_name(dt), s2 ? 1 : 0, ch.mt, ch.nw,
                   conv_deep_ring_depth(dt, ch.mt, ch.nw, (Cin / 32) * 9 + (a.res_mode == 2 ? (a.RCA + a.RCB) / 32 : 0), ch.nb),
                   ch.nb);
        L.ops.back().kinst = ki;
      }
      {
        auto base = L.ops.back().run;
        ConvArgs a0 = a;
        L.ops.back().run_dbg = [lp, ctx, a0, s2, ch, dt, B, temb, toff](hipStream_t s, int fl) {
          ConvArgs x = a0;
          if (temb && !(fl & 4)) { x.temb = lp->rs.temb + toff; x.temb_ld = ctx->SC; x.temb_per_b = lp->rs.temb_per_b; x.t_dev = lp->rs.t_dev; }
          if (fl & 1) x.stats = nullptr;
          if (fl & 2) x.gamma = nullptr;
          if (fl & 4) x.res_mode = 0;
          x.dbg = fl;
          if (ch.strip) return launch_conv_strip(dt, ch.nblk, ch.mpi, ch.SR, x, B, s);
          if (ch.tile >= 0) return launch_conv_tile(dt, ch.tile, s2, x, B, s);
          x.deep_zin = deep_zin(x, B, dtype_size(dt)); x.deep_nw = ch.nw; x.deep_nb = ch.nb;
          return launch_conv_deep(dt, ch.mt, s2, x, B, s);
        };
        (void)base;
      }
    } else {
      FinalArgs f{};
      const Tensor src = TT(st.srcA);
      f.src = src.p; f.C = src.C;
      {
        const GNRes& gr = gres[st.gn];
        const Tensor ga = TT(gr.a);
        f.gst = ga.stats; f.gtiles = ga.tiles; f.gntile = ga.n_tile;
        f.gamma = WF("final_conv.gamma"); f.beta = WF("final_conv.beta"); f.groups = u.groups; f.eps = 1e-5f;
        if (ga.C % u.groups || 256 % u.groups) FAIL(SDDM_ERR_SHAPE, "final GroupNorm grouping");
      }
      f.w = WF("final_conv.w");
      f.bias = c->params.at("final_conv.block.3.bias").data[0];
      static const int env_ft = std::getenv("SDDM_FINAL_FT") ? std::atoi(std::getenv("SDDM_FINAL_FT")) : 0;
      f.N = N; f.F = F; f.W = W; f.S = S; f.FT = (env_ft == 16 && F % 16 == 0) ? 16 : (F % 8 == 0 ? 8 : 2);
      if (F % f.FT || W % S) FAIL(SDDM_ERR_SHAPE, "final tile: frames %d, segment %d/%d", F, W, S);
      f.co = c->coef();
      const double bytes = (double)B * F * W * src.C * es + (double)B * N * 4 * 3;
      const double flops = 2.0 * B * F * W * src.C * 9;
#ifdef SDDM_STAMPS
      if (const char* sn = std::getenv("SDDM_STAMPS"))
        if (std::string(sn) == "final_conv") {
          if (!c->stamp_buf) SDDM_HIP_CHECK(hipMalloc(&c->stamp_buf, sizeof(unsigned long long) * 8 * 65536));
          f.stamps = c->stamp_buf;
          c->stamp_blocks = (int64_t)(F / f.FT) * B;
        }
#endif
      L.ops.push_back({3, bytes, flops, [lp, f, dt, B](hipStream_t s) {
                          FinalArgs x = f;
                          x.mode = lp->rs.final_mode; x.eps_out = lp->rs.eps_out;
                          x.x = lp->rs.x; x.cond = lp->rs.cond; x.t_dev = lp->rs.t_dev;
                          x.seed = lp->rs.seed; x.row_offset = lp->rs.row_offset;
                          x.noise = lp->rs.noise; x.noise_ld = lp->rs.noise_ld;
                          x.sp = lp->rs.t_dev ? (const StepParams*)lp->rs.t_dev : nullptr;
                          return launch_final(dt, x, B, s);
                        }, "final_conv"});
      L.ops.back().kname = std::string("final_kernel<") + dt_name(dt) + (f.FT >= 16 ? ",1024>" : ",512>");
      L.ops.back().kinst = L.ops.back().kname;
    }
  }
  return SDDM_OK;
}

static int build_plan(sddm_ctx* c, int B) {
  c->lanes.clear();
  c->plan_B = -1;
  const int LR = std::max(1, c->lane_rows);
  const int nl = (B + LR - 1) / LR;
  if (nl > kMaxLanes) FAIL(SDDM_ERR_INVALID_ARG, "batch %d needs %d lanes (max %d): raise SDDM_LANE_ROWS", B, nl, kMaxLanes);
  for (int l = 0; l < nl; ++l) {
    std::unique_ptr<Lane> L(new Lane());
    L->idx = l;
    L->row0 = l * LR;
    L->B = std::min(LR, B - l * LR);
    const int r = build_lane(c, *L);
    if (r) { c->lanes.clear(); return r; }
    c->lanes.push_back(std::move(L));
  }
  c->plan_B = B;
  c->plan_gen++;
  return SDDM_OK;
}

static int ensure_ready(sddm_ctx* c) {
  if (!c || !c->configured) FAIL(SDDM_ERR_STATE, "context not configured");
  if (c->net_type.empty()) FAIL(SDDM_ERR_STATE, "context has no network (diffusion-only)");
  SDDM_HIP_CHECK(hipSetDevice(c->device));
  for (const auto& kv : c->params)
    if (!kv.second.loaded) FAIL(SDDM_ERR_STATE, "parameter %s not loaded", kv.first.c_str());
  if (c->params_dirty) {
    const int r = c->dws ? dw_upload_weights(c) : (c->wgs ? wg_upload_weights(c) : (c->wus ? wu_upload_weights(c) : upload_weights(c)));
    if (r) return r;
  }
  if (c->tables_dirty) {
    const int r = upload_tables(c);
    if (r) return r;
  }
  return SDDM_OK;
}

static int prof_drain(sddm_ctx* c, const Lane& L) {
  if (c->ev_pend.empty()) return SDDM_OK;
  SDDM_HIP_CHECK(hipEventSynchronize(c->ev_pool[c->ev_pend.back().second + 1]));
  if (c->op_acc.size() < L.ops.size()) c->op_acc.resize(L.ops.size());
  for (const auto& pe : c->ev_pend) {
    float m = 0;
    SDDM_HIP_CHECK(hipEventElapsedTime(&m, c->ev_pool[pe.second], c->ev_pool[pe.second + 1]));
    ProfAcc& a = c->op_acc[pe.first];
    a.ms += m; a.n += 1; a.bytes += L.ops[pe.first].bytes; a.flops += L.ops[pe.first].flops;
  }
  c->ev_pend.clear();
  return SDDM_OK;
}

static int run_ops(sddm_ctx* c, Lane& L, hipStream_t s) {
  for (const Op& op : L.ops) {
    const bool timed = c->prof && c->ev_pend.size() * 2 + 2 <= c->ev_pool.size();
    int e0 = 0;
    if (timed) {
      e0 = (int)c->ev_pend.size() * 2;
      SDDM_HIP_CHECK(hipEventRecord(c->ev_pool[e0], s));
    }
    hipError_t e = op.run(s);
    if (e != hipSuccess) FAIL(SDDM_ERR_HIP, "kernel launch failed: %s", hipGetErrorString(e));
    {
      static const char* rop = std::getenv("SDDM_REPEAT_OP");
      static const int rn = std::getenv("SDDM_REPEAT_N") ? std::atoi(std::getenv("SDDM_REPEAT_N")) : 0;
      static const int rflags = std::getenv("SDDM_REPEAT_FLAGS") ? std::atoi(std::getenv("SDDM_REPEAT_FLAGS")) : 0;
      if (rop && op.name.rfind(rop, 0) == 0)
        for (int k = 0; k < rn && e == hipSuccess; ++k) e = (rflags && op.run_dbg) ? op.run_dbg(s, rflags) : op.run(s);
      if (e != hipSuccess) FAIL(SDDM_ERR_HIP, "kernel launch failed: %s", hipGetErrorString(e));
    }
    if (timed) {
      SDDM_HIP_CHECK(hipEventRecord(c->ev_pool[e0 + 1], s));
      c->ev_pend.push_back({(int)(&op - L.ops.data()), e0});
    }
  }
  if (c->prof) return prof_drain(c, L);
  return SDDM_OK;
}

extern "C" {

int sddm_abi_version(void) { return SDDM_ABI_VERSION; }
const char* sddm_last_error(void) { return g_last_error.c_str(); }

int sddm_create(int device, int compute_dtype, sddm_ctx** out) {
  if (!out) FAIL(SDDM_ERR_INVALID_ARG, "out is NULL");
  if (compute_dtype < 0 || compute_dtype > 2) FAIL(SDDM_ERR_INVALID_ARG, "bad dtype %d", compute_dtype);
  int n = 0;
  if (hipGetDeviceCount(&n) != hipSuccess || device < 0 || device >= n)
    FAIL(SDDM_ERR_HIP, "no HIP device %d (count %d)", device, n);
  int lds = 0;
  if (hipDeviceGetAttribute(&lds, hipDeviceAttributeMaxSharedMemoryPerBlock, device) != hipSuccess || lds < kLdsBytes)
    FAIL(SDDM_ERR_HIP, "device %d offers %d bytes of LDS per workgroup; the kernels are planned for %d (gfx950)", device,
         lds, kLdsBytes);
  sddm_ctx* c = new sddm_ctx();
  c->device = device;
  c->dtype = compute_dtype;
  c->use_graphs = std::getenv("SDDM_NO_GRAPH") == nullptr;
  if (const char* lr = std::getenv("SDDM_LANE_ROWS")) c->lane_rows = std::max(1, std::atoi(lr));
  *out = c;
  return SDDM_OK;
}

void sddm_destroy(sddm_ctx* c) {
  if (!c) return;
  (void)hipSetDevice(c->device);
  for (int k = 0; k < kStreams; ++k) {
    if (c->work[k]) { (void)hipStreamSynchronize(c->work[k]); (void)hipStreamDestroy(c->work[k]); }
    if (c->ev_done[k]) (void)hipEventDestroy(c->ev_done[k]);
  }
  c->lanes.clear();
  if (c->dws) c->dws->act.reset();
  if (c->wgs) c->wgs->act.reset();
  if (c->wus) c->wus->act.reset();
  if (c->ev_in) (void)hipEventDestroy(c->ev_in);
  for (hipEvent_t e : c->ev_pool) (void)hipEventDestroy(e);
  c->warena.reset();
  delete c;
}

int sddm_schedule(const char* schedule, int n_timestep, double linear_start, double linear_end, float* out) {
  if (!schedule || !out || n_timestep < 1) FAIL(SDDM_ERR_INVALID_ARG, "bad schedule arguments");
  if (compute_schedule(schedule, n_timestep, linear_start, linear_end, out))
    FAIL(SDDM_ERR_NOT_IMPLEMENTED, "schedule '%s'", schedule);
  return SDDM_OK;
}

int sddm_configure(sddm_ctx* c, const char* json) {
  if (!c || !json) FAIL(SDDM_ERR_INVALID_ARG, "NULL argument");
  Json cfg;
  try {
    cfg = Json::parse(json);
  } catch (const std::exception& e) {
    FAIL(SDDM_ERR_INVALID_ARG, "config JSON: %s", e.what());
  }
  const Json& arch = cfg.at("arch");
  const Json& diff = cfg.at("diffusion");
  const Json& net = cfg.at("network");
  c->arch_type = arch.string("type", "SDDM");
  if (!std::getenv("SDDM_LANE_ROWS")) {
    const int lr = (int)cfg.number("lane_rows", 16);
    if (lr < 1) FAIL(SDDM_ERR_INVALID_ARG, "lane_rows %d", lr);
    c->lane_rows = lr;
    c->plan_B = -1;
  }
  const Json& aa = arch.at("args");
  const std::string nc = aa.string("noise_condition", "sqrt_alpha_bar");
  if (nc != "sqrt_alpha_bar" && nc != "time_step") FAIL(SDDM_ERR_NOT_IMPLEMENTED, "noise_condition '%s'", nc.c_str());
  c->noise_time_step = nc == "time_step";
  if (c->arch_type == "SDDM") {
    const std::string pt = aa.string("p_transition", "original");
    const std::string qt = aa.string("q_transition", "original");
    if (pt == "original") { c->tr_mode = SDDM_TR_ORIGINAL; c->init_mode = 0; }
    else if (pt == "condition_in") { c->tr_mode = SDDM_TR_ORIGINAL; c->init_mode = 4; }
    else if (pt == "sr3") { c->tr_mode = SDDM_TR_SR3; c->init_mode = 1; }
    else if (pt == "supportive") { c->tr_mode = SDDM_TR_SUPPORTIVE; c->init_mode = 2; }
    else if (pt == "conditional") { c->tr_mode = SDDM_TR_CONDITIONAL; c->init_mode = 3; }
    else FAIL(SDDM_ERR_NOT_IMPLEMENTED, "p_transition '%s' (model.py:20-23)", pt.c_str());
    if (qt != "original" && qt != "conditional") FAIL(SDDM_ERR_NOT_IMPLEMENTED, "q_transition '%s'", qt.c_str());
    c->p_transition = pt;
  } else if (c->arch_type == "SDDM_spectrogram") {
    c->tr_mode = SDDM_TR_ORIGINAL;
    c->init_mode = 0;
    c->p_transition = "original";
    c->hop_samples = (int)aa.number("hop_samples", 256);
    if (c->hop_samples < 1) FAIL(SDDM_ERR_INVALID_ARG, "hop_samples %d", c->hop_samples);
  } else {
    FAIL(SDDM_ERR_NOT_IMPLEMENTED, "arch type '%s'", c->arch_type.c_str());
  }
  if (diff.string("type", "GaussianDiffusion") != "GaussianDiffusion")
    FAIL(SDDM_ERR_NOT_IMPLEMENTED, "diffusion type '%s'", diff.string("type", "").c_str());
  const Json& da = diff.at("args");
  const std::string sched = da.string("schedule", "linear");
  const int T = (int)da.number("n_timestep", 1000);
  const double ls = da.number("linear_start", 1e-4), le = da.number("linear_end", 2e-2);
  if (T < 1) FAIL(SDDM_ERR_INVALID_ARG, "n_timestep %d", T);
  std::vector<float> tabs((size_t)14 * (T + 1));
  if (compute_schedule(sched, T, ls, le, tabs.data())) FAIL(SDDM_ERR_NOT_IMPLEMENTED, "schedule '%s' (diffusion.py:84)", sched.c_str());
  c->net_type = net.string("type", "");
  if (c->net_type.empty()) {
    c->T = T;
    c->tables.swap(tabs);
    c->tables_dirty = true;
    c->params.clear();
    c->plan_B = -1;
    c->lanes.clear();
    c->warena.reset();
    c->configured = true;
    return SDDM_OK;
  }
  if (c->net_type == "DiffWave") {
    if (c->arch_type != "SDDM_spectrogram") FAIL(SDDM_ERR_NOT_IMPLEMENTED, "DiffWave needs arch SDDM_spectrogram");
    const Json& na = net.at("args");
    auto d = std::make_shared<DWState>();
    d->C = (int)na.number("residual_channels", 64);
    d->L = (int)na.number("residual_layers", 30);
    d->cycle = (int)na.number("dilation_cycle_length", 10);
    d->bins = (int)na.number("freq_bins", na.number("stft_bins", na.number("n_mels", 513)));
    d->hop = c->hop_samples;
    d->Kp = (d->bins + 31) / 32 * 32;
    if (d->C != 64) FAIL(SDDM_ERR_NOT_IMPLEMENTED, "DiffWave residual_channels %d (kernels are built for 64)", d->C);
    if (d->L < 1 || d->cycle < 1 || d->bins < 1) FAIL(SDDM_ERR_INVALID_ARG, "DiffWave geometry");
    if (d->hop != 256) FAIL(SDDM_ERR_NOT_IMPLEMENTED, "hop_samples %d: SpectrogramUpsampler upsamples x256", d->hop);
    c->T = T;
    c->tables.swap(tabs);
    c->tables_dirty = true;
    c->num_samples = -1;
    c->params.clear();
    for (const auto& kv : dw_param_shapes(*d)) {
      Param p;
      p.shape = kv.second;
      c->params[kv.first] = p;
    }
    c->params["diffusion_embedding.embedding_vector"].loaded = true;
    c->dws = d;
    c->wgs.reset();
    c->wus.reset();
    c->params_dirty = true;
    c->plan_B = -1;
    c->lanes.clear();
    c->warena.reset();
    c->configured = true;
    return SDDM_OK;
  }
  if (const wg::Variant* wv = wg::find_variant(c->net_type)) {
    if (wv->kind == wg::kWaveGrad) {
      if (c->arch_type != "SDDM_spectrogram") FAIL(SDDM_ERR_NOT_IMPLEMENTED, "WaveGrad needs arch SDDM_spectrogram");
      if (c->hop_samples != wv->hop)
        FAIL(SDDM_ERR_NOT_IMPLEMENTED, "hop_samples %d: WaveGrad upsamples x300 (config_wavegrad.json:8)", c->hop_samples);
    } else {
      if (c->arch_type != "SDDM") FAIL(SDDM_ERR_NOT_IMPLEMENTED, "%s needs arch SDDM (its condition is a waveform)", wv->name);
      c->hop_samples = wv->hop;
    }
    c->T = T;
    c->tables.swap(tabs);
    c->tables_dirty = true;
    c->num_samples = -1;
    c->params.clear();
    auto ws = std::make_shared<WGState>();
    ws->v = wv;
    ws->shapes = wg_param_shapes(*wv);
    for (const auto& kv : ws->shapes) {
      Param p;
      p.shape = kv.second;
      c->params[kv.first] = p;
    }
    c->dws.reset();
    c->wgs = ws;
    c->wus.reset();
    c->params_dirty = true;
    c->plan_B = -1;
    c->lanes.clear();
    c->warena.reset();
    c->configured = true;
    return SDDM_OK;
  }
  if (c->net_type == "Waveunet3") {
    if (c->arch_type != "SDDM") FAIL(SDDM_ERR_NOT_IMPLEMENTED, "Waveunet3 needs arch SDDM (its condition is a waveform)");
    const int r = wu_check_config(net.at("args"));
    if (r) return r;
    c->T = T;
    c->tables.swap(tabs);
    c->tables_dirty = true;
    c->num_samples = -1;
    c->params.clear();
    auto us = std::make_shared<WUState>();
    us->shapes = wu_param_shapes(us->net);
    for (const auto& kv : us->shapes) {
      Param p;
      p.shape = kv.second;
      c->params[kv.first] = p;
    }
    c->dws.reset();
    c->wgs.reset();
    c->wus = us;
    c->params_dirty = true;
    c->plan_B = -1;
    c->lanes.clear();
    c->warena.reset();
    c->configured = true;
    return SDDM_OK;
  }
  if (c->net_type != "UNetModified2") FAIL(SDDM_ERR_NOT_IMPLEMENTED, "network type '%s'", c->net_type.c_str());
  if (c->arch_type != "SDDM") FAIL(SDDM_ERR_NOT_IMPLEMENTED, "UNetModified2 under arch '%s'", c->arch_type.c_str());
  c->dws.reset();
  c->wgs.reset();
  c->wus.reset();
  const Json& na = net.at("args");
  UNetCfg u;
  u.in_channel = (int)na.number("in_channel", 2);
  u.out_channel = (int)na.number("out_channel", 1);
  u.inner = (int)na.number("inner_channel", 32);
  u.groups = (int)na.number("norm_groups", 32);
  u.mults = na.ints("channel_mults", {1, 2, 3, 4, 5});
  u.res_blocks = (int)na.number("res_blocks", 3);
  u.dropout = na.number("dropout", 0.0);
  u.seg = (int)na.number("segment_len", 128);
  u.stride = (int)na.number("segment_stride", 64);
  const int Ns = (int)cfg.number("num_samples", (double)na.number("num_samples", -1));
  if (u.in_channel != 2 || u.out_channel != 1)
    FAIL(SDDM_ERR_NOT_IMPLEMENTED, "UNetModified2 with in_channel %d / out_channel %d", u.in_channel, u.out_channel);
  if (u.inner > 128 || u.inner % 32) FAIL(SDDM_ERR_NOT_IMPLEMENTED, "inner_channel %d (multiples of 32 up to 128)", u.inner);
  if (Ns <= u.seg || (Ns - u.seg) % u.stride) FAIL(SDDM_ERR_SHAPE, "num_samples %d: (n - %d) %% %d != 0 (UNetModified2.py:13)", Ns, u.seg, u.stride);
  const int F = (Ns - u.seg) / u.stride + 1;
  const int div = 1 << (int)u.mults.size();
  if (F % div || u.seg % div) FAIL(SDDM_ERR_SHAPE, "n_frames %d and segment_len %d must be multiples of %d", F, u.seg, div);
  if (u.seg % u.stride) FAIL(SDDM_ERR_NOT_IMPLEMENTED, "segment_len %% segment_stride != 0");
  c->T = T;
  c->tables.swap(tabs);
  c->tables_dirty = true;
  c->ucfg = u;
  c->num_samples = Ns;
  c->params.clear();
  for (const auto& kv : unet_param_shapes(u)) {
    Param p;
    p.shape = kv.second;
    c->params[kv.first] = p;
  }
  c->params_dirty = true;
  c->plan_B = -1;
  c->lanes.clear();
  c->warena.reset();
  c->configured = true;
  return SDDM_OK;
}

int sddm_load_param(sddm_ctx* c, const char* key_c, const void* host_ptr, const int64_t* shape, int ndim,
                    int src_dtype) {
  if (!c || !c->configured) FAIL(SDDM_ERR_STATE, "context not configured");
  if (!key_c || !host_ptr || (ndim > 0 && !shape)) FAIL(SDDM_ERR_INVALID_ARG, "NULL argument");
  std::string key = key_c;
  if (key.rfind("module.", 0) == 0) key = key.substr(7);
  int64_t n = 1;
  for (int i = 0; i < ndim; ++i) n *= shape[i];
  auto read = [&](std::vector<float>& dst) -> int {
    dst.resize((size_t)n);
    if (src_dtype == DT_F32) std::memcpy(dst.data(), host_ptr, sizeof(float) * n);
    else if (src_dtype == DT_BF16) {
      for (int64_t i = 0; i < n; ++i) {
        uint32_t u = (uint32_t)((const uint16_t*)host_ptr)[i] << 16;
        std::memcpy(&dst[i], &u, 4);
      }
    } else if (src_dtype == DT_F16) {
      for (int64_t i = 0; i < n; ++i) dst[i] = (float)((const _Float16*)host_ptr)[i];
    } else {
      return 1;
    }
    return 0;
  };
  if (key.rfind("diffusion.", 0) == 0) {
    const std::string name = key.substr(10);
    for (int k = 0; k < 14; ++k)
      if (name == kTableNames[k]) {
        if (ndim != 1 || shape[0] != c->T + 1)
          FAIL(SDDM_ERR_SHAPE, "%s: expected [%d]", key.c_str(), c->T + 1);
        std::vector<float> v;
        if (read(v)) FAIL(SDDM_ERR_INVALID_ARG, "bad src dtype %d", src_dtype);
        std::memcpy(c->tables.data() + (size_t)k * (c->T + 1), v.data(), sizeof(float) * v.size());
        c->tables_dirty = true;
        return SDDM_OK;
      }
    FAIL(SDDM_ERR_INVALID_ARG, "unexpected key %s", key.c_str());
  }
  if (key.rfind("noise_estimate_model.", 0) == 0) key = key.substr(21);
  auto it = c->params.find(key);
  if (it == c->params.end()) FAIL(SDDM_ERR_INVALID_ARG, "unexpected key %s", key_c);
  Param& p = it->second;
  if ((int)p.shape.size() != ndim) FAIL(SDDM_ERR_SHAPE, "%s: rank %d != %d", key_c, ndim, (int)p.shape.size());
  for (int i = 0; i < ndim; ++i)
    if (p.shape[i] != shape[i]) FAIL(SDDM_ERR_SHAPE, "%s: shape mismatch in dim %d", key_c, i);
  if (read(p.data)) FAIL(SDDM_ERR_INVALID_ARG, "bad src dtype %d", src_dtype);
  p.loaded = true;
  c->params_dirty = true;
  return SDDM_OK;
}

int sddm_missing_params(sddm_ctx* c, int64_t* n_missing) {
  if (!c || !n_missing) FAIL(SDDM_ERR_INVALID_ARG, "NULL argument");
  int64_t m = 0;
  for (const auto& kv : c->params) m += kv.second.loaded ? 0 : 1;
  *n_missing = m;
  return SDDM_OK;
}

static int prepare_plan(sddm_ctx* c, int64_t B, int64_t N) {
  if (N != c->num_samples)
    FAIL(SDDM_ERR_SHAPE, "condition has %lld samples, network built for num_samples=%d", (long long)N, c->num_samples);
  if (B < 1 || B > 65535) FAIL(SDDM_ERR_INVALID_ARG, "batch %lld", (long long)B);
  if (c->plan_B != (int)B) return build_plan(c, (int)B);
  return SDDM_OK;
}

static int sample_impl(sddm_ctx* c, const float* cond, int64_t B, int64_t N, uint64_t seed, int64_t row_offset,
                       float* out, float* record, int sample_inter, void* stream, const float* noise = nullptr);

int sddm_sample(sddm_ctx* c, const float* cond, int64_t B, int64_t N, uint64_t seed, int64_t row_offset,
                float* out, void* stream) {
  return sample_impl(c, cond, B, N, seed, row_offset, out, nullptr, 0, stream);
}

int sddm_sample_noise(sddm_ctx* c, const float* cond, int64_t B, int64_t N, const float* noise, float* out,
                      void* stream) {
  if (!noise) FAIL(SDDM_ERR_INVALID_ARG, "NULL noise");
  return sample_impl(c, cond, B, N, 0, 0, out, nullptr, 0, stream, noise);
}

int sddm_sample_continuous(sddm_ctx* c, const float* cond, int64_t B, int64_t N, uint64_t seed,
                           int64_t row_offset, float* out, float* record, int sample_inter, void* stream) {
  if (!record || sample_inter < 1) FAIL(SDDM_ERR_INVALID_ARG, "record buffer / sample_inter");
  return sample_impl(c, cond, B, N, seed, row_offset, out, record, sample_inter, stream);
}

static int sample_impl(sddm_ctx* c, const float* cond, int64_t B, int64_t N, uint64_t seed, int64_t row_offset,
                       float* out, float* record, int sample_inter, void* stream, const float* noise) {
  int r = ensure_ready(c);
  if (r) return r;
  if (!cond || !out) FAIL(SDDM_ERR_INVALID_ARG, "NULL tensor");
  if (c->dws) return dw_sample(c, cond, B, N, seed, row_offset, out, record, sample_inter, noise, (hipStream_t)stream);
  if (c->wgs) return wg_sample(c, cond, B, N, seed, row_offset, out, record, sample_inter, noise, (hipStream_t)stream);
  if (c->wus) return wu_sample(c, cond, B, N, seed, row_offset, out, record, sample_inter, noise, (hipStream_t)stream);
  r = prepare_plan(c, B, N);
  if (r) return r;
  hipStream_t user = (hipStream_t)stream;
  const bool graph = c->use_graphs && !c->prof && !record && !noise;
  const int T = c->T;
  StepParams* sp0 = c->warena.at<StepParams>(c->off_tdev);
  float* temb_tab = c->warena.at<float>(c->off_temb_tab);
  EmbedArgs e{};
  e.table = c->dtab(3); e.time_step_mode = c->noise_time_step; e.R = T + 1; e.dim = c->ucfg.inner;
  e.emb_vec = c->warena.at<float>(c->woff.at("emb_vec"));
  e.w1 = c->warena.at<float>(c->woff.at("mlp.w1")); e.b1 = c->warena.at<float>(c->woff.at("mlp.b1"));
  e.w2 = c->warena.at<float>(c->woff.at("mlp.w2")); e.b2 = c->warena.at<float>(c->woff.at("mlp.b2"));
  e.pw = c->warena.at<float>(c->woff.at("proj.w")); e.pb = c->warena.at<float>(c->woff.at("proj.b"));
  e.SC = c->SC; e.out = temb_tab;
  SDDM_HIP_CHECK(launch_embed(e, user));
  for (auto& Lp : c->lanes) {
    Lane& L = *Lp;
    const int64_t rows = L.B, off = (int64_t)L.row0 * N;
    float* xb = graph ? L.arena.at<float>(L.off_x) : out + off;
    const float* cb = cond + off;
    if (graph) {
      SDDM_HIP_CHECK(hipMemcpyAsync(L.arena.at<float>(L.off_cond), cb, sizeof(float) * rows * N,
                                    hipMemcpyDeviceToDevice, user));
      cb = L.arena.at<float>(L.off_cond);
    }
    StepParams* sp = (StepParams*)((char*)sp0 + 64 * L.idx);
    InitArgs ia{};
    ia.mode = c->init_mode; ia.cond = cb; ia.out = xb; ia.total = rows * N; ia.N = N; ia.T = T;
    ia.co = c->coef(); ia.seed = seed; ia.row_offset = row_offset + L.row0;
    ia.noise = noise ? noise + off : nullptr;
    SDDM_HIP_CHECK(launch_init_state(ia, user));
    SDDM_HIP_CHECK(launch_set_params(sp, T + 1, seed, row_offset + L.row0, user));
    L.rs.cond = cb; L.rs.x = xb; L.rs.temb = temb_tab; L.rs.temb_per_b = 0; L.rs.t_dev = &sp->t;
    L.rs.final_mode = c->tr_mode; L.rs.eps_out = nullptr; L.rs.seed = seed; L.rs.row_offset = row_offset + L.row0;
    L.rs.noise = noise ? noise + off : nullptr; L.rs.noise_ld = B * N;
  }
  if (graph) {
    const int ns = std::min<int>(kStreams, (int)c->lanes.size());
    if (!c->ev_in) SDDM_HIP_CHECK(hipEventCreateWithFlags(&c->ev_in, hipEventDisableTiming));
    for (int k = 0; k < ns; ++k)
      if (!c->work[k]) {
        SDDM_HIP_CHECK(hipStreamCreateWithFlags(&c->work[k], hipStreamNonBlocking));
        SDDM_HIP_CHECK(hipEventCreateWithFlags(&c->ev_done[k], hipEventDisableTiming));
      }
    SDDM_HIP_CHECK(hipEventRecord(c->ev_in, user));
    for (int k = 0; k < ns; ++k) SDDM_HIP_CHECK(hipStreamWaitEvent(c->work[k], c->ev_in, 0));
    int K = 1;
    for (int k : {10, 8, 5, 4, 2})
      if (T % k == 0) { K = k; break; }
    for (auto& Lp : c->lanes) {
      Lane& L = *Lp;
      if (L.gexec && L.g_gen == c->plan_gen && L.g_K == K) continue;
      if (L.gexec) { (void)hipGraphExecDestroy(L.gexec); L.gexec = nullptr; }
      if (L.graph) { (void)hipGraphDestroy(L.graph); L.graph = nullptr; }
      hipStream_t s = c->work[L.idx % ns];
      SDDM_HIP_CHECK(hipStreamBeginCapture(s, hipStreamCaptureModeThreadLocal));
      for (int k = 0; k < K; ++k) {
        r = run_ops(c, L, s);
        if (r) {
          hipGraph_t junk = nullptr;
          (void)hipStreamEndCapture(s, &junk);
          if (junk) (void)hipGraphDestroy(junk);
          return r;
        }
      }
      SDDM_HIP_CHECK(hipStreamEndCapture(s, &L.graph));
      SDDM_HIP_CHECK(hipGraphInstantiate(&L.gexec, L.graph, nullptr, nullptr, 0));
      L.g_gen = c->plan_gen;
      L.g_K = K;
    }
    static const int off_us = std::getenv("SDDM_LANE_OFFSET_US") ? std::atoi(std::getenv("SDDM_LANE_OFFSET_US")) : 0;
    if (off_us > 0)
      for (auto& Lp : c->lanes)
        if (Lp->idx % ns) SDDM_HIP_CHECK(launch_delay((unsigned)(off_us * (Lp->idx % ns)), c->work[Lp->idx % ns]));
    for (int i = 0; i < T / K; ++i)
      for (auto& Lp : c->lanes) SDDM_HIP_CHECK(hipGraphLaunch(Lp->gexec, c->work[Lp->idx % ns]));
    for (auto& Lp : c->lanes)
      SDDM_HIP_CHECK(hipMemcpyAsync(out + (int64_t)Lp->row0 * N, Lp->rs.x, sizeof(float) * Lp->B * N,
                                    hipMemcpyDeviceToDevice, c->work[Lp->idx % ns]));
    for (int k = 0; k < ns; ++k) {
      SDDM_HIP_CHECK(hipEventRecord(c->ev_done[k], c->work[k]));
      SDDM_HIP_CHECK(hipStreamWaitEvent(user, c->ev_done[k], 0));
    }
    return SDDM_OK;
  }
  int64_t nrec = 0;
  for (int t = T; t >= 1; --t) {
    for (auto& Lp : c->lanes) {
      r = run_ops(c, *Lp, user);
      if (r) return r;
    }
    if (record && t % sample_inter == 0) {
      SDDM_HIP_CHECK(hipMemcpyAsync(record + nrec * B * N, out, sizeof(float) * B * N, hipMemcpyDeviceToDevice, user));
      ++nrec;
    }
  }
  return SDDM_OK;
}

int sddm_network_forward(sddm_ctx* c, const float* cond, const float* x_t, const float* noise_level, int64_t B,
                         int64_t N, float* eps_out, void* stream) {
  int r = ensure_ready(c);
  if (r) return r;
  if (!cond || !x_t || !noise_level || !eps_out) FAIL(SDDM_ERR_INVALID_ARG, "NULL tensor");
  if (c->dws) return dw_forward(c, cond, x_t, noise_level, B, N, eps_out, (hipStream_t)stream);
  if (c->wgs) return wg_forward(c, cond, x_t, noise_level, B, N, eps_out, (hipStream_t)stream);
  if (c->wus) return wu_forward(c, cond, x_t, noise_level, B, N, eps_out, (hipStream_t)stream);
  r = prepare_plan(c, B, N);
  if (r) return r;
  hipStream_t s = (hipStream_t)stream;
  for (auto& Lp : c->lanes) {
    Lane& L = *Lp;
    const int64_t off = (int64_t)L.row0 * N;
    float* temb = L.arena.at<float>(L.off_temb_fwd);
    EmbedArgs e{};
    e.noise_levels = noise_level + L.row0; e.R = L.B; e.dim = c->ucfg.inner;
    e.emb_vec = c->warena.at<float>(c->woff.at("emb_vec"));
    e.w1 = c->warena.at<float>(c->woff.at("mlp.w1")); e.b1 = c->warena.at<float>(c->woff.at("mlp.b1"));
    e.w2 = c->warena.at<float>(c->woff.at("mlp.w2")); e.b2 = c->warena.at<float>(c->woff.at("mlp.b2"));
    e.pw = c->warena.at<float>(c->woff.at("proj.w")); e.pb = c->warena.at<float>(c->woff.at("proj.b"));
    e.SC = c->SC; e.out = temb;
    SDDM_HIP_CHECK(launch_embed(e, s));
    L.rs.cond = cond + off; L.rs.x = const_cast<float*>(x_t) + off; L.rs.temb = temb; L.rs.temb_per_b = 1;
    L.rs.t_dev = nullptr; L.rs.final_mode = -1; L.rs.eps_out = eps_out + off; L.rs.seed = 0; L.rs.row_offset = 0;
    L.rs.noise = nullptr;
    r = run_ops(c, L, s);
    if (r) return r;
  }
  return SDDM_OK;
}

int sddm_transition(sddm_ctx* c, int mode, const float* x_t, const float* eps, const float* cond, int t, int64_t B,
                    int64_t N, uint64_t seed, int64_t row_offset, float* out, void* stream) {
  if (!c || !c->configured) FAIL(SDDM_ERR_STATE, "context not configured");
  if (mode < 0 || mode > 4) FAIL(SDDM_ERR_NOT_IMPLEMENTED, "transition mode %d", mode);
  if (t < 1 || t > c->T) FAIL(SDDM_ERR_INVALID_ARG, "t=%d outside [1, %d]", t, c->T);
  if (!x_t || !eps || !out || (mode >= 2 && mode <= 3 && !cond)) FAIL(SDDM_ERR_INVALID_ARG, "NULL tensor");
  SDDM_HIP_CHECK(hipSetDevice(c->device));
  if (!c->warena.base) {
    c->warena.reset();
    c->off_tables = c->warena.reserve(sizeof(float) * 14 * (c->T + 1));
    c->off_tdev = c->warena.reserve(64 * kMaxLanes);
    SDDM_HIP_CHECK(c->warena.commit());
    c->params_dirty = true;
    c->tables_dirty = true;
  }
  if (c->tables_dirty) {
    const int r = upload_tables(c);
    if (r) return r;
  }
  TransArgs a{};
  a.mode = mode; a.x_t = x_t; a.eps = eps; a.cond = cond; a.out = out; a.total = B * N; a.N = N; a.t = t;
  a.co = c->coef(); a.seed = seed; a.row_offset = row_offset;
  SDDM_HIP_CHECK(launch_transition(a, (hipStream_t)stream));
  return SDDM_OK;
}

int sddm_q_sample(sddm_ctx* c, int mode, const float* x0, const float* y, const float* noise, const int64_t* t,
                  const float* r, int64_t B, int64_t N, float* x_t, float* combined, float* s_out, float* level_out,
                  void* stream) {
  if (!c || !c->configured) FAIL(SDDM_ERR_STATE, "context not configured");
  if (mode < 0 || mode > 1) FAIL(SDDM_ERR_NOT_IMPLEMENTED, "q_sample mode %d", mode);
  if (!x0 || !noise || !t || !x_t || (mode == 1 && !y)) FAIL(SDDM_ERR_INVALID_ARG, "NULL tensor");
  if (B < 0 || N < 1) FAIL(SDDM_ERR_INVALID_ARG, "shape B=%lld N=%lld", (long long)B, (long long)N);
  SDDM_HIP_CHECK(hipSetDevice(c->device));
  if (!c->warena.base) {
    c->warena.reset();
    c->off_tables = c->warena.reserve(sizeof(float) * 14 * (c->T + 1));
    c->off_tdev = c->warena.reserve(64 * kMaxLanes);
    SDDM_HIP_CHECK(c->warena.commit());
    c->params_dirty = true;
    c->tables_dirty = true;
  }
  if (c->tables_dirty) {
    const int rr = upload_tables(c);
    if (rr) return rr;
  }
  QArgs a{};
  a.mode = mode; a.x0 = x0; a.y = y; a.noise = noise; a.t = t; a.r = r;
  a.sab = c->dtab(3); a.alpha_bar = c->dtab(2); a.m = c->dtab(8); a.sqrt_delta = c->dtab(9);
  a.x_t = x_t; a.combined = combined; a.s_out = s_out; a.level_out = level_out; a.B = B; a.N = N;
  SDDM_HIP_CHECK(launch_q_sample(a, (hipStream_t)stream));
  return SDDM_OK;
}

int sddm_set_conv_tuning(sddm_ctx* c, const char* json) {
  if (!c || !json) FAIL(SDDM_ERR_INVALID_ARG, "NULL argument");
  Json j;
  try {
    j = Json::parse(json);
  } catch (const std::exception& e) {
    FAIL(SDDM_ERR_INVALID_ARG, "tuning JSON: %s", e.what());
  }
  std::vector<const Json*> tabs;
  if (j.has("tables")) {
    const Json& arr = j.at("tables");
    if (arr.kind != Json::ARR) FAIL(SDDM_ERR_INVALID_ARG, "tables: a list");
    for (const auto& t : arr.arr) tabs.push_back(&t);
  } else {
    tabs.push_back(&j);
  }
  std::vector<sddm_ctx::TuneTable> out;
  for (const Json* tp : tabs) {
    const Json& t = *tp;
    if (t.kind != Json::OBJ) FAIL(SDDM_ERR_INVALID_ARG, "tuning table: an object");
    sddm_ctx::TuneTable tt;
    const std::string dts = t.string("dtype", "");
    tt.dtype = dts == "float32" ? DT_F32 : dts == "bfloat16" ? DT_BF16 : dts == "float16" ? DT_F16 : -1;
    if (t.has("deep"))
      for (const auto& kv : t.at("deep").obj) {
        if (kv.second.kind != Json::ARR || kv.second.arr.size() != 2) FAIL(SDDM_ERR_INVALID_ARG, "deep.%s: [mt, nw]", kv.first.c_str());
        tt.deep_tune[kv.first] = {(int)kv.second.arr[0].num, (int)kv.second.arr[1].num};
      }
    if (t.has("kernel"))
      for (const auto& kv : t.at("kernel").obj) {
        if (kv.second.kind != Json::STR) FAIL(SDDM_ERR_INVALID_ARG, "kernel.%s: a string", kv.first.c_str());
        const std::string& v = kv.second.str;
        sddm_ctx::KernTune k{0, 0, 0, 0};
        if (v == "strip") k.kind = 1;
        else if (v.rfind("tile:", 0) == 0) { k.kind = 2; k.a = std::atoi(v.c_str() + 5); }
        else if (v == "deep") k.kind = 3;
        else if (v.rfind("deep:", 0) == 0) { k.kind = 3; std::sscanf(v.c_str() + 5, "%d:%d:%d", &k.a, &k.b, &k.c); }
        else if (v == "chain") k.kind = 4;
        else FAIL(SDDM_ERR_INVALID_ARG, "kernel.%s: unknown choice '%s'", kv.first.c_str(), v.c_str());
        if (k.kind == 2 && (k.a < 0 || k.a >= conv_tile_ncfg())) FAIL(SDDM_ERR_INVALID_ARG, "kernel.%s: tile configuration %d", kv.first.c_str(), k.a);
        tt.kern_tune[kv.first] = k;
      }
    tt.B = (int)t.number("lane_batch", -1);
    tt.N = (int)t.number("num_samples", -1);
    out.push_back(std::move(tt));
  }
  c->tunes = std::move(out);
  c->plan_B = -1;
  c->lanes.clear();
  return SDDM_OK;
}

int sddm_log_spectrogram(const float* audio, int64_t B, int64_t N, int n_fft, int hop, const float* window,
                         const float* fb, int n_out, float* out, void* stream) {
  if (!audio || !window || !out) FAIL(SDDM_ERR_INVALID_ARG, "NULL tensor");
  if (n_fft < 2 || n_fft > 1024 || (n_fft & (n_fft - 1))) FAIL(SDDM_ERR_NOT_IMPLEMENTED, "n_fft %d (powers of two <= 1024)", n_fft);
  if (hop < 1 || B < 1 || N <= n_fft / 2) FAIL(SDDM_ERR_SHAPE, "B=%lld N=%lld hop=%d n_fft=%d", (long long)B, (long long)N, hop, n_fft);
  if (!fb && n_out != n_fft / 2 + 1) FAIL(SDDM_ERR_INVALID_ARG, "linear spectrogram has %d bins, not %d", n_fft / 2 + 1, n_out);
  StftArgs a{};
  a.audio = audio; a.B = B; a.N = N; a.n_fft = n_fft; a.hop = hop; a.frames = (int)(1 + N / hop); a.n_out = n_out;
  a.window = window; a.fb = fb; a.out = out;
  SDDM_HIP_CHECK(launch_stft_features(a, (hipStream_t)stream));
  return SDDM_OK;
}

int sddm_initial_state(sddm_ctx* c, int mode, const float* cond, int64_t B, int64_t N, uint64_t seed,
                       int64_t row_offset, float* out, void* stream) {
  if (!c || !c->configured) FAIL(SDDM_ERR_STATE, "context not configured");
  if (mode < 0 || mode > 4) FAIL(SDDM_ERR_NOT_IMPLEMENTED, "init mode %d", mode);
  if (!out || (mode >= 2 && !cond)) FAIL(SDDM_ERR_INVALID_ARG, "NULL tensor");
  SDDM_HIP_CHECK(hipSetDevice(c->device));
  if (!c->warena.base) {
    c->warena.reset();
    c->off_tables = c->warena.reserve(sizeof(float) * 14 * (c->T + 1));
    c->off_tdev = c->warena.reserve(64 * kMaxLanes);
    SDDM_HIP_CHECK(c->warena.commit());
    c->params_dirty = true;
    c->tables_dirty = true;
  }
  if (c->tables_dirty) {
    const int r = upload_tables(c);
    if (r) return r;
  }
  InitArgs ia{};
  ia.mode = mode; ia.cond = cond; ia.out = out; ia.total = B * N; ia.N = N; ia.T = c->T;
  ia.co = c->coef(); ia.seed = seed; ia.row_offset = row_offset;
  SDDM_HIP_CHECK(launch_init_state(ia, (hipStream_t)stream));
  return SDDM_OK;
}

int sddm_profile_enable(sddm_ctx* c, int enable) {
  if (!c) FAIL(SDDM_ERR_INVALID_ARG, "NULL ctx");
  SDDM_HIP_CHECK(hipSetDevice(c->device));
  c->prof = enable != 0;
  c->ev_pend.clear();
  c->op_acc.clear();
  if (c->prof && c->ev_pool.empty()) {
    c->ev_pool.resize(512);
    for (auto& e : c->ev_pool) SDDM_HIP_CHECK(hipEventCreate(&e));
  }
  return SDDM_OK;
}

static const std::vector<Op>& profiled_ops(sddm_ctx* c) {
  static const std::vector<Op> kNoOps;
  return c->lanes.empty() ? kNoOps : c->lanes[0]->ops;
}

int sddm_profile_read(sddm_ctx* c, const char* kernel_class, double* avg_ms, int64_t* launches,
                      double* bytes_per_launch, double* flops_per_launch) {
  if (!c || !kernel_class) FAIL(SDDM_ERR_INVALID_ARG, "NULL argument");
  const std::string k = kernel_class;
  const int cls = k == "conv_in" ? 0 : k == "gn_finalize" ? 1 : k == "conv3x3" ? 2 : k == "final" ? 3 : -1;
  if (cls < 0) FAIL(SDDM_ERR_INVALID_ARG, "kernel class %s", kernel_class);
  const std::vector<Op>& ops = profiled_ops(c);
  double ms = 0, bytes = 0, flops = 0;
  int64_t n = 0;
  for (size_t i = 0; i < c->op_acc.size() && i < ops.size(); ++i) {
    if (ops[i].cls != cls) continue;
    ms += c->op_acc[i].ms; bytes += c->op_acc[i].bytes; flops += c->op_acc[i].flops; n += c->op_acc[i].n;
  }
  if (avg_ms) *avg_ms = n ? ms / n : 0.0;
  if (launches) *launches = n;
  if (bytes_per_launch) *bytes_per_launch = n ? bytes / n : 0.0;
  if (flops_per_launch) *flops_per_launch = n ? flops / n : 0.0;
  return SDDM_OK;
}

int sddm_debug_stamps(sddm_ctx* c, void* host, int64_t max_blocks, int64_t* n_blocks) {
  if (!c || !host || !n_blocks) FAIL(SDDM_ERR_INVALID_ARG, "NULL argument");
  *n_blocks = 0;
  if (!c->stamp_buf) return SDDM_OK;
  const int64_t n = std::min<int64_t>(c->stamp_blocks, max_blocks);
  SDDM_HIP_CHECK(hipDeviceSynchronize());
  SDDM_HIP_CHECK(hipMemcpy(host, c->stamp_buf, sizeof(unsigned long long) * 8 * n, hipMemcpyDeviceToHost));
  *n_blocks = n;
  return SDDM_OK;
}

int sddm_profile_ops(sddm_ctx* c, char* buf, int64_t buflen) {
  if (!c || !buf || buflen < 3) FAIL(SDDM_ERR_INVALID_ARG, "NULL argument");
  const std::vector<Op>& ops = profiled_ops(c);
  std::string js = "[";
  char tmp[768];
  for (size_t i = 0; i < ops.size(); ++i) {
    const ProfAcc a = i < c->op_acc.size() ? c->op_acc[i] : ProfAcc{};
    snprintf(tmp, sizeof(tmp),
             "%s{\"name\": \"%s\", \"kernel\": \"%s\", \"inst\": \"%s\", \"cls\": %d, \"launches\": %lld, "
             "\"avg_ms\": %.6f, \"bytes\": %.0f, \"flops\": %.0f}",
             i ? ", " : "", ops[i].name.c_str(), ops[i].kname.c_str(), ops[i].kinst.c_str(), ops[i].cls, (long long)a.n,
             a.n ? a.ms / a.n : 0.0, ops[i].bytes, ops[i].flops);
    js += tmp;
  }
  js += "]";
  if ((int64_t)js.size() + 1 > buflen) FAIL(SDDM_ERR_INVALID_ARG, "buffer too small (%zu)", js.size() + 1);
  std::memcpy(buf, js.c_str(), js.size() + 1);
  return SDDM_OK;
}

}
```

### speech-denoising-diffusion-model-2_amd/sddm_hip/__init__.py

```python
import ctypes
import json
import os

import numpy as np

HERE = os.path.dirname(os.path.abspath(__file__))
LIB_PATH = os.environ.get("SDDM_LIB") or os.path.join(HERE, "libsddm_hip.so")

OK, ERR_NOT_IMPLEMENTED, ERR_INVALID_ARG, ERR_SHAPE, ERR_HIP, ERR_STATE = range(6)
F32, BF16, F16 = 0, 1, 2
TR_ORIGINAL, TR_SR3, TR_SUPPORTIVE, TR_CONDITIONAL, TR_CONDITION_IN = range(5)
DTYPES = {"float32": F32, "fp32": F32, "f32": F32, "bfloat16": BF16, "bf16": BF16,
          "float16": F16, "fp16": F16, "f16": F16}
TRANSITIONS = {"original": TR_ORIGINAL, "condition_in": TR_CONDITION_IN, "sr3": TR_SR3,
               "supportive": TR_SUPPORTIVE, "conditional": TR_CONDITIONAL}
TABLE_NAMES = ("betas", "alphas", "alpha_bar", "sqrt_alpha_bar", "predicted_noise_coeff", "sigma",
               "supportive_gamma", "supportive_sigma_hat", "m", "sqrt_delta", "c_xt", "c_yt", "c_epst",
               "sqrt_delta_estimated")
EXPORTS = ("sddm_abi_version", "sddm_last_error", "sddm_create", "sddm_destroy", "sddm_configure",
           "sddm_load_param", "sddm_missing_params", "sddm_sample", "sddm_sample_noise", "sddm_sample_continuous",
           "sddm_network_forward",
           "sddm_transition", "sddm_q_sample", "sddm_log_spectrogram", "sddm_set_conv_tuning", "sddm_initial_state", "sddm_schedule", "sddm_profile_enable",
           "sddm_profile_read", "sddm_profile_ops")

_lib = None


def lib():
    global _lib
    if _lib is None:
        if not os.path.exists(LIB_PATH):
            raise RuntimeError(f"{LIB_PATH} not built: run __graft_entry__.build() or "
                               "python speech-denoising-diffusion-model-2_amd/sddm_hip/build.py")
        L = ctypes.CDLL(LIB_PATH)
        vp, i64, u64, c_int = ctypes.c_void_p, ctypes.c_int64, ctypes.c_uint64, ctypes.c_int
        L.sddm_abi_version.restype = c_int
        L.sddm_last_error.restype = ctypes.c_char_p
        L.sddm_create.argtypes = [c_int, c_int, ctypes.POINTER(vp)]
        L.sddm_destroy.argtypes = [vp]
        L.sddm_destroy.restype = None
        L.sddm_configure.argtypes = [vp, ctypes.c_char_p]
        L.sddm_load_param.argtypes = [vp, ctypes.c_char_p, vp, ctypes.POINTER(i64), c_int, c_int]
        L.sddm_missing_params.argtypes = [vp, ctypes.POINTER(i64)]
        L.sddm_sample.argtypes = [vp, vp, i64, i64, u64, i64, vp, vp]
        L.sddm_sample_noise.argtypes = [vp, vp, i64, i64, vp, vp, vp]
        L.sddm_sample_continuous.argtypes = [vp, vp, i64, i64, u64, i64, vp, vp, c_int, vp]
        L.sddm_network_forward.argtypes = [vp, vp, vp, vp, i64, i64, vp, vp]
        L.sddm_transition.argtypes = [vp, c_int, vp, vp, vp, c_int, i64, i64, u64, i64, vp, vp]
        L.sddm_q_sample.argtypes = [vp, c_int, vp, vp, vp, vp, vp, i64, i64, vp, vp, vp, vp, vp]
        L.sddm_log_spectrogram.argtypes = [vp, i64, i64, c_int, c_int, vp, vp, c_int, vp, vp]
        L.sddm_set_conv_tuning.argtypes = [vp, ctypes.c_char_p]
        L.sddm_initial_state.argtypes = [vp, c_int, vp, i64, i64, u64, i64, vp, vp]
        L.sddm_schedule.argtypes = [ctypes.c_char_p, c_int, ctypes.c_double, ctypes.c_double, vp]
        L.sddm_profile_enable.argtypes = [vp, c_int]
        L.sddm_profile_read.argtypes = [vp, ctypes.c_char_p, ctypes.POINTER(ctypes.c_double),
                                        ctypes.POINTER(i64), ctypes.POINTER(ctypes.c_double),
                                        ctypes.POINTER(ctypes.c_double)]
        L.sddm_profile_ops.argtypes = [vp, ctypes.c_char_p, i64]
        for name in EXPORTS:
            if name not in ("sddm_last_error", "sddm_destroy", "sddm_abi_version"):
                getattr(L, name).restype = c_int
        _lib = L
    return _lib


class SddmError(RuntimeError):
    pass


def check(status):
    if status == OK:
        return
    msg = lib().sddm_last_error().decode(errors="replace")
    if status == ERR_NOT_IMPLEMENTED:
        raise NotImplementedError(msg)
    if status == ERR_SHAPE:
        raise AssertionError(msg)
    if status == ERR_INVALID_ARG:
        raise ValueError(msg)
    raise SddmError(f"sddm status {status}: {msg}")


def schedule(schedule="linear", n_timestep=1000, linear_start=1e-4, linear_end=2e-2):
    out = np.empty((14, int(n_timestep) + 1), dtype=np.float32)
    check(lib().sddm_schedule(str(schedule).encode(), int(n_timestep), float(linear_start),
                              float(linear_end), out.ctypes.data))
    return dict(zip(TABLE_NAMES, out))


def _ptr(t):
    return ctypes.c_void_p(0 if t is None else t.data_ptr())


def _stream(torch, device):
    return ctypes.c_void_p(torch.cuda.current_stream(device).cuda_stream)


class Context:

    def __init__(self, config, device=0, compute_dtype="float32"):
        self.device = int(device)
        self.dtype = DTYPES[str(compute_dtype)]
        h = ctypes.c_void_p()
        check(lib().sddm_create(self.device, self.dtype, ctypes.byref(h)))
        self._h = h
        check(lib().sddm_configure(self._h, json.dumps(config).encode()))
        self.timesteps = int(config.get("diffusion", {}).get("args", {}).get("n_timestep", 1000))

    def close(self):
        if getattr(self, "_h", None):
            lib().sddm_destroy(self._h)
            self._h = None

    def __del__(self):
        try:
            self.close()
        except Exception:
            pass

    def load_param(self, key, array):
        a = np.ascontiguousarray(np.asarray(array, dtype=np.float32))
        shape = (ctypes.c_int64 * max(a.ndim, 1))(*a.shape)
        check(lib().sddm_load_param(self._h, key.encode(), a.ctypes.data, shape, a.ndim, F32))

    def load_state_dict(self, state):
        for k, v in state.items():
            if hasattr(v, "detach"):
                v = v.detach().float().cpu().numpy()
            self.load_param(k, v)

    def missing(self):
        n = ctypes.c_int64()
        check(lib().sddm_missing_params(self._h, ctypes.byref(n)))
        return n.value

    def sample(self, cond, out, seed, row_offset=0):
        import torch
        B, N = out.shape[0], out.shape[-1]
        check(lib().sddm_sample(self._h, _ptr(cond), B, N, int(seed) & (2 ** 64 - 1), int(row_offset),
                                _ptr(out), _stream(torch, cond.device)))

    def sample_noise(self, cond, out, noise):
        import torch
        B, N = out.shape[0], out.shape[-1]
        T = self.timesteps
        if not isinstance(noise, torch.Tensor) or noise.dtype != torch.float32 or not noise.is_contiguous():
            raise ValueError("noise must be a contiguous float32 tensor")
        if noise.device != out.device:
            raise ValueError(f"noise must be on {out.device}, got {noise.device}")
        if noise.dim() < 2 or noise.shape[1] != B or noise.shape[0] != T + 1 or \
                noise.numel() != noise.shape[0] * B * N:
            raise ValueError(f"noise must be [T + 1, {B}, {N}] draws, got {tuple(noise.shape)}")
        check(lib().sddm_sample_noise(self._h, _ptr(cond), B, N, _ptr(noise), _ptr(out), _stream(torch, cond.device)))

    def sample_continuous(self, cond, out, record, sample_inter, seed, row_offset=0):
        import torch
        B, N = out.shape[0], out.shape[-1]
        check(lib().sddm_sample_continuous(self._h, _ptr(cond), B, N, int(seed) & (2 ** 64 - 1),
                                           int(row_offset), _ptr(out), _ptr(record), int(sample_inter),
                                           _stream(torch, cond.device)))

    def network_forward(self, cond, x_t, noise_level, eps_out):
        import torch
        B, N = x_t.shape[0], x_t.shape[-1]
        check(lib().sddm_network_forward(self._h, _ptr(cond), _ptr(x_t), _ptr(noise_level), B, N,
                                         _ptr(eps_out), _stream(torch, cond.device)))

    def transition(self, mode, x_t, eps, cond, t, out, seed, row_offset=0):
        import torch
        B, N = x_t.shape[0], x_t.numel() // x_t.shape[0]
        check(lib().sddm_transition(self._h, int(mode), _ptr(x_t), _ptr(eps), _ptr(cond), int(t), B, N,
                                    int(seed) & (2 ** 64 - 1), int(row_offset), _ptr(out),
                                    _stream(torch, x_t.device)))

    def set_conv_tuning(self, table):
        import json as _json
        text = table if isinstance(table, str) else _json.dumps(table)
        check(lib().sddm_set_conv_tuning(self._h, text.encode()))

    def q_sample(self, mode, x0, y, noise, t, r, x_t, combined, s_out, level_out):
        import torch
        B, N = x0.shape[0], x0.numel() // x0.shape[0]
        check(lib().sddm_q_sample(self._h, int(mode), _ptr(x0), _ptr(y), _ptr(noise), _ptr(t), _ptr(r), B, N,
                                  _ptr(x_t), _ptr(combined), _ptr(s_out), _ptr(level_out),
                                  _stream(torch, x0.device)))

    def initial_state(self, mode, cond, out, seed, row_offset=0):
        import torch
        B, N = out.shape[0], out.numel() // out.shape[0]
        check(lib().sddm_initial_state(self._h, int(mode), _ptr(cond), B, N, int(seed) & (2 ** 64 - 1),
                                       int(row_offset), _ptr(out), _stream(torch, out.device)))

    def profile(self, enable=True):
        check(lib().sddm_profile_enable(self._h, 1 if enable else 0))

    def profile_read(self, kernel_class):
        ms, b, f = ctypes.c_double(), ctypes.c_double(), ctypes.c_double()
        n = ctypes.c_int64()
        check(lib().sddm_profile_read(self._h, kernel_class.encode(), ctypes.byref(ms), ctypes.byref(n),
                                      ctypes.byref(b), ctypes.byref(f)))
        return dict(avg_ms=ms.value, launches=n.value, bytes_per_launch=b.value, flops_per_launch=f.value)

    def profile_ops(self):
        buf = ctypes.create_string_buffer(1 << 20)
        check(lib().sddm_profile_ops(self._h, buf, len(buf)))
        return json.loads(buf.value.decode())


def log_spectrogram(audio, n_fft, hop, window, fb, n_out, out):
    import torch
    B, N = audio.shape
    check(lib().sddm_log_spectrogram(_ptr(audio), B, N, int(n_fft), int(hop), _ptr(window), _ptr(fb), int(n_out),
                                     _ptr(out), _stream(torch, audio.device)))
```

### speech-denoising-diffusion-model-2_amd/sddm_hip/build.py

```python
import concurrent.futures as cf
import glob
import os
import subprocess
import sys

HERE = os.path.dirname(os.path.abspath(__file__))
PKG = os.path.dirname(HERE)
CSRC = os.path.join(PKG, "csrc")
INCLUDE = os.path.join(os.path.dirname(PKG), "include")
VARIANT = os.environ.get("SDDM_BUILD_VARIANT", "")
if VARIANT:
    _OUT = os.path.join(os.path.dirname(PKG), "tools", "_" + VARIANT)
    BUILD = os.path.join(_OUT, "_build")
    LIB = os.path.join(_OUT, "libsddm_hip.so")
else:
    BUILD = os.path.join(HERE, "_build")
    LIB = os.path.join(HERE, "libsddm_hip.so")
SOURCES = ["kernels.hip", "conv_strip.hip", "conv_strip_bf16.hip", "conv_strip_f16.hip", "conv_strip_f32.hip", "conv_deep.hip", "conv_tile.hip", "conv_chain.hip", "diffwave.hip", "wavegrad.hip", "waveunet.hip", "q_sample.hip", "stft.hip", "sddm_runtime.cpp",
           "schedule.cpp"]
HIPCC = os.environ.get("HIPCC", "/opt/rocm/bin/hipcc")
ARCH = os.environ.get("SDDM_OFFLOAD_ARCH", "gfx950")
FLAGS = ["-O3", "-std=c++17", "-fPIC", f"--offload-arch={ARCH}", "-I", CSRC, "-I", INCLUDE,
         "-Wno-unused-result"] + (["-DSDDM_STAMPS"] if VARIANT.startswith("stamps") else [])
if VARIANT:
    FLAGS += os.environ.get("SDDM_EXTRA_DEFS", "").split()


def _deps(path, seen=None):
    import re
    seen = set() if seen is None else seen
    with open(path) as f:
        for name in re.findall(r'^\s*#\s*include\s+"([^"]+)"', f.read(), re.M):
            for d in (CSRC, INCLUDE):
                h = os.path.join(d, name)
                if os.path.exists(h) and h not in seen:
                    seen.add(h)
                    _deps(h, seen)
    return sorted(seen)


def _stale(target, inputs):
    if not os.path.exists(target):
        return True
    t = os.path.getmtime(target)
    return any(os.path.getmtime(i) > t for i in inputs)


def _compile(src):
    obj = os.path.join(BUILD, os.path.basename(src) + ".o")
    if _stale(obj, [os.path.join(CSRC, src)] + _deps(os.path.join(CSRC, src))):
        cmd = [HIPCC] + FLAGS + ["-c", os.path.join(CSRC, src), "-o", obj]
        r = subprocess.run(cmd, capture_output=True, text=True)
        if r.returncode != 0:
            raise RuntimeError(f"hipcc failed for {src}:\n{r.stdout}\n{r.stderr}")
    return obj


def build(verbose=False):
    os.makedirs(BUILD, exist_ok=True)
    with cf.ThreadPoolExecutor(max_workers=len(SOURCES)) as ex:
        objs = list(ex.map(_compile, SOURCES))
    if _stale(LIB, objs):
        cmd = [HIPCC, "-shared", f"--offload-arch={ARCH}", "-Wl,--no-undefined", "-o", LIB] + objs
        r = subprocess.run(cmd, capture_output=True, text=True)
        if r.returncode != 0:
            raise RuntimeError(f"link failed:\n{r.stdout}\n{r.stderr}")
    if verbose:
        print("built", LIB)
    return LIB


if __name__ == "__main__":
    build(verbose=True)
    sys.exit(0)
```

Before: 25.78 audio_s/s.

## Fold nearest upsample into 3x3 conv via polyphase 2x2 weights

Adds a phase-decomposed path for nearest-upsample-then-3x3 convolutions. Each of the four output phases becomes a 2x2 conv over the low-resolution source, using precomputed summed weights (16 taps instead of 9 per output). This reads half-width source rows into the LDS ring and does 4 MACs per output instead of 9, cutting upsample-conv FLOPs and LDS traffic. It needs extra phase weight tensors (w_p, w_pt, w_pf) and is enabled by default for non-f32 dtypes, with different rounding from summing weights first.

```diff
diff --git a/include/sddm_hip.h b/include/sddm_hip.h
--- a/include/sddm_hip.h
+++ b/include/sddm_hip.h
@@ -73,6 +73,8 @@
 int sddm_schedule(const char* schedule, int n_timestep, double linear_start, double linear_end,
                   float* out);
 
+int sddm_upsample_phase_weights(const float* w, int cout, int cin, float* out16);
+
 int sddm_profile_enable(sddm_ctx* ctx, int enable);
 int sddm_profile_read(sddm_ctx* ctx, const char* kernel_class, double* avg_ms, int64_t* launches,
                       double* bytes_per_launch, double* flops_per_launch);
diff --git a/speech-denoising-diffusion-model-2_amd/csrc/conv_strip_impl.h b/speech-denoising-diffusion-model-2_amd/csrc/conv_strip_impl.h
--- a/speech-denoising-diffusion-model-2_amd/csrc/conv_strip_impl.h
+++ b/speech-denoising-diffusion-model-2_amd/csrc/conv_strip_impl.h
@@ -51,7 +51,7 @@
          a.Hi == (c.up ? c.Ho / 2 : c.Ho) && a.Wi == (c.up ? c.Wo / 2 : c.Wo);
 }
 
-template <typename T, int FC, int W, int CIN, int MPI, int RES, bool GN, int SH>
+template <typename T, int FC, int W, int CIN, int MPI, int RES, bool GN, int SH, bool PH = false>
 __global__ __launch_bounds__(MPI * 2) void conv_strip_kernel(ConvArgs a, int SR_) {
   constexpr ConvShape SC = kStripShapes[SH];
   constexpr bool CS = SH > 0;
@@ -62,22 +62,30 @@
   constexpr int NWV = NT / 64;
   constexpr int ES = (int)sizeof(T);
   constexpr int NBLK = 16 * FC, FP = 2;
-  constexpr int TR = MPI / W, R = 2 * TR + 2;
+  constexpr int TR = MPI / W;
+  constexpr int WR = PH ? W / 2 : W, TRr = PH ? TR / 2 : TR;
+  constexpr int R = 2 * TRr + 2;
+  constexpr int NTAP = PH ? 16 : 9;
+  constexpr int NTW = PH ? 8 : 9;
+  static_assert(!PH || (TR % 2 == 0 && WR % 16 == 0 && RES == 0 && !GN), "phase path: plain Upsample convs, whole source rows");
   constexpr int UPP = CIN * ES / 16;
   constexpr int UPL = ES / 2;
   constexpr int VE = 16 / ES;
-  constexpr int PL = ((W + 2) * 16 + 255) / 256 * 256;
+  constexpr int PL = ((WR + 2) * 16 + 255) / 256 * 256;
   constexpr int SLOT = UPP * PL;
   constexpr int NCK = CIN / 32;
   constexpr int WPL = NBLK * 16;
-  constexpr int WPLANES = NCK * 9 * 4 * UPL;
+  constexpr int WPLANES = NCK * NTAP * 4 * UPL;
   constexpr int PB = 64 / UPP;
-  constexpr int NU = TR * W * UPP;
-  constexpr int UPT = NU / NT;
-  constexpr int IU = ((TR + 2) * W * UPP + NT - 1) / NT;
+  constexpr int NU = TRr * WR * UPP;
+  constexpr int UPT = (NU + NT - 1) / NT;
+  constexpr bool RAG = NU % NT != 0;
+  constexpr int NINI = (TRr + 2) * WR * UPP;
+  constexpr int IU = (NINI + NT - 1) / NT;
   constexpr int RCKM = 4;
   static_assert(UPP >= 1 && UPP <= 64 && (64 % UPP) == 0, "channel units must divide a wave");
-  static_assert(NU % NT == 0, "prefetch must split evenly");
+  static_assert(PH || NU % NT == 0, "prefetch must split evenly");
+  static_assert(NU % 64 == 0, "prefetch units fill whole waves");
   typedef T vec4 __attribute__((ext_vector_type(4)));
   extern __shared__ __attribute__((aligned(16))) char smem[];
 
@@ -86,6 +94,8 @@
   xcd_block<SDDM_XCD_ZIN != 0>(gNT, gCout / NBLK, strip, b, zb);
   const int n0 = zb * NBLK;
   const int H = gHo;
+  const int Hr = PH ? gHi : gHo;
+  const bool up_map = gUp && !PH;
   const int RC = gRCA + gRCB;
   const int rck = RES == 2 ? RC / 32 : 0;
   constexpr bool gn = GN;
@@ -98,6 +108,7 @@
   float* red = gsc + 2 * CIN;
 
   const int y0 = strip * SR;
+  const int y0r = PH ? y0 / 2 : y0;
   const int iters = SR / TR;
   SDDM_STAMP(a, 0);
   GNLoad gl;
@@ -108,17 +119,17 @@
   f32x4 ini[IU];
 #pragma unroll
   for (int k = 0; k < IU; ++k) {
-    const int u = min(tid + k * NT, (TR + 2) * W * UPP - 1);
+    const int u = min(tid + k * NT, NINI - 1);
     const int grp = u >> 6, j = u & 63;
-    const int pix = grp * PB + (j % PB), q = j / PB, r = pix / W, x = pix % W;
-    const int ry = min(max(y0 - 1 + r, 0), H - 1);
-    const int sy = gUp ? ry >> 1 : ry, sx = gUp ? x >> 1 : x;
+    const int pix = grp * PB + (j % PB), q = j / PB, r = pix / WR, x = pix % WR;
+    const int ry = min(max(y0r - 1 + r, 0), Hr - 1);
+    const int sy = up_map ? ry >> 1 : ry, sx = up_map ? x >> 1 : x;
     const int c0 = q * VE;
     const bool fa = c0 < gCA;
     ini[k] = *(const f32x4*)((fa ? srcAb : srcBb) + ((size_t)sy * gWi + sx) * (fa ? gCA : gCB) + (fa ? c0 : c0 - gCA));
   }
   constexpr int WUN = NBLK * WPLANES, WU = (WUN + NT - 1) / NT;
-  constexpr bool WLD = SDDM_STRIP_WLD && WU <= 12;
+  constexpr bool WLD = SDDM_STRIP_WLD && WU <= (PH ? 16 : 12);
   constexpr int RUN_MAX = RES == 2 ? NBLK * RCKM * 4 * UPL : 0, RU = (RUN_MAX + NT - 1) / NT;
   const int RUN = NBLK * RPLANES;
   f32x4 wst[WLD ? WU : 1], rst[WLD && RU > 0 ? RU : 1];
@@ -131,8 +142,8 @@
       if constexpr (ES == 2) {
         src = (const char*)a.wgt_t + ((size_t)pl * gCout + n0 + co) * 16;
       } else {
-        const int ck = pl / (9 * 4 * UPL), rem = pl - ck * 9 * 4 * UPL, tap = rem / (4 * UPL), un = rem - tap * 4 * UPL;
-        src = (const char*)a.wgt + ((((size_t)(n0 + co) * NCK + ck) * 9 + tap) * 32) * ES + un * 16;
+        const int ck = pl / (NTAP * 4 * UPL), rem = pl - ck * NTAP * 4 * UPL, tap = rem / (4 * UPL), un = rem - tap * 4 * UPL;
+        src = (const char*)a.wgt + ((((size_t)(n0 + co) * NCK + ck) * NTAP + tap) * 32) * ES + un * 16;
       }
       wst[i] = *(const f32x4*)src;
     }
@@ -154,8 +165,8 @@
       if constexpr (ES == 2) {
         src = (const char*)a.wgt_t + ((size_t)pl * gCout + n0 + co) * 16;
       } else {
-        const int ck = pl / (9 * 4 * UPL), rem = pl - ck * 9 * 4 * UPL, tap = rem / (4 * UPL), un = rem - tap * 4 * UPL;
-        src = (const char*)a.wgt + ((((size_t)(n0 + co) * NCK + ck) * 9 + tap) * 32) * ES + un * 16;
+        const int ck = pl / (NTAP * 4 * UPL), rem = pl - ck * NTAP * 4 * UPL, tap = rem / (4 * UPL), un = rem - tap * 4 * UPL;
+        src = (const char*)a.wgt + ((((size_t)(n0 + co) * NCK + ck) * NTAP + tap) * 32) * ES + un * 16;
       }
       __builtin_amdgcn_global_load_lds((const __attribute__((address_space(1))) void*)src,
                                        (__attribute__((address_space(3))) void*)(wl + u0 * 16), 16, 0, 0);
@@ -173,7 +184,7 @@
   }
   for (int u = tid; u < R * UPP * 2; u += NT) {
     const int side = u & 1, pl = u >> 1;
-    *(f32x4*)(ring + pl * PL + (side ? (W + 1) : 0) * 16) = f32x4{0.f, 0.f, 0.f, 0.f};
+    *(f32x4*)(ring + pl * PL + (side ? (WR + 1) : 0) * 16) = f32x4{0.f, 0.f, 0.f, 0.f};
   }
   if (gn) gl.finish(gf, b, gCA, gCB, gsc, gsc + CIN);
   __syncthreads();
@@ -194,16 +205,16 @@
     const float bv = a.bias[cs], tv = trow[cs];
     sshift = bv + (a.temb ? tv : 0.f);
   }
-  const int base = ((y0 - 1) % R + R) % R;
+  const int base = ((y0r - 1) % R + R) % R;
 #pragma unroll
   for (int k = 0; k < IU; ++k) {
     const int u = tid + k * NT;
-    if (u >= (TR + 2) * W * UPP) break;
+    if (u >= NINI) break;
     const int grp = u >> 6, j = u & 63;
-    const int pix = grp * PB + (j % PB), q = j / PB, r = pix / W, x = pix % W;
-    const int ry = y0 - 1 + r;
+    const int pix = grp * PB + (j % PB), q = j / PB, r = pix / WR, x = pix % WR;
+    const int ry = y0r - 1 + r;
     f32x4 v = ini[k];
-    if (ry < 0 || ry >= H) v = f32x4{0.f, 0.f, 0.f, 0.f};
+    if (ry < 0 || ry >= Hr) v = f32x4{0.f, 0.f, 0.f, 0.f};
     else if (gn) v = transform_fast<T>(v, gsc + q * VE, gsc + CIN + q * VE);
     *(f32x4*)(ring + ((base + r) % R) * SLOT + q * PL + (x + 1) * 16) = v;
   }
@@ -222,24 +233,30 @@
   static_assert(W % 32 == 0, "a wave's 32 pixels must not cross rows");
   const int wave_u = __builtin_amdgcn_readfirstlane(wave);
   int prow[FP], pcol[FP];
+  const int py = wave_u & 1, srow = ((wave_u >> 1) * 16) / WR, scol = ((wave_u >> 1) * 16) % WR + (lane & 15);
 #pragma unroll
   for (int fp = 0; fp < FP; ++fp) {
-    prow[fp] = (wave_u * 32) / W;
-    pcol[fp] = (wave_u * 32) % W + fp * 16 + (lane & 15);
+    if constexpr (PH) {
+      prow[fp] = 2 * srow + py;
+      pcol[fp] = 2 * scol + fp;
+    } else {
+      prow[fp] = (wave_u * 32) / W;
+      pcol[fp] = (wave_u * 32) % W + fp * 16 + (lane & 15);
+    }
   }
   int pr[UPT], loff[UPT], cq[UPT];
   const char* rsrc_[UPT];
   unsigned rstr[UPT];
 #pragma unroll
   for (int k = 0; k < UPT; ++k) {
-    const int u = tid + k * NT, grp = u >> 6, j = u & 63;
+    const int u = RAG ? min(tid + k * NT, NU - 1) : tid + k * NT, grp = u >> 6, j = u & 63;
     const int pix = grp * PB + (j % PB);
-    const int q = j / PB, x = pix % W;
-    pr[k] = pix / W;
+    const int q = j / PB, x = pix % WR;
+    pr[k] = pix / WR;
     loff[k] = q * PL + (x + 1) * 16;
     cq[k] = q * VE;
     const int c0 = q * VE;
-    const int sx = gUp ? (x >> 1) : x;
+    const int sx = up_map ? (x >> 1) : x;
     const bool fa = c0 < gCA;
     rsrc_[k] = fa ? (const char*)(srcAb + sx * gCA + c0) : (const char*)(srcBb + sx * gCB + (c0 - gCA));
     rstr[k] = (unsigned)(gWi * (fa ? gCA : gCB) * ES);
@@ -247,21 +264,22 @@
   auto issue_rows = [&](f32x4 (&dst)[UPT], int j) {
 #pragma unroll
     for (int k = 0; k < UPT; ++k) {
-      const int ry = min(y0 + j * TR + 1 + pr[k], H - 1);
-      const int sy = gUp ? (ry >> 1) : ry;
+      const int ry = min(y0r + j * TRr + 1 + pr[k], Hr - 1);
+      const int sy = up_map ? (ry >> 1) : ry;
       dst[k] = *(const f32x4*)(rsrc_[k] + (unsigned)__umul24((unsigned)sy, rstr[k]));
     }
   };
   auto xform_unit = [&](const f32x4 (&src)[UPT], int j, int k) {
-    const int ry = y0 + j * TR + 1 + pr[k];
+    const int ry = y0r + j * TRr + 1 + pr[k];
     f32x4 v = src[k];
     if constexpr (GN) v = transform_lds<T>(v, gsc + cq[k], gsc + CIN + cq[k]);
-    return ry >= H ? f32x4{0.f, 0.f, 0.f, 0.f} : v;
+    return ry >= Hr ? f32x4{0.f, 0.f, 0.f, 0.f} : v;
   };
   auto store_rows = [&](const f32x4 (&tv)[UPT], int j) {
-    const int sb = (base + j * TR + 2) % R;
+    const int sb = (base + j * TRr + 2) % R;
 #pragma unroll
     for (int k = 0; k < UPT; ++k) {
+      if (RAG && tid + k * NT >= NU) continue;
       int sl = sb + pr[k];
       sl = sl >= R ? sl - R : sl;
       *(f32x4*)(ring + (int)__umul24(sl, SLOT) + loff[k]) = tv[k];
@@ -309,11 +327,11 @@
   vec4 r1A[FP][FC], r1B[FP][FC];
   Frag<T> r2A[RCKM][FP], r2B[RCKM][FP];
   constexpr bool WREG = SDDM_STRIP_WREG && ES == 2 && NCK == 1 && FC == 2 && RES != 2 && MPI == 256;
-  Frag<T> wreg[WREG ? 9 : 1][FC];
+  Frag<T> wreg[WREG ? NTW : 1][FC];
   auto body = [&](auto LR, auto LX, int it, f32x4 (&nxt)[UPT], f32x4 (&fill)[UPT], vec4 (&r1cur)[FP][FC],
                   vec4 (&r1nxt)[FP][FC], Frag<T> (&r2cur)[RCKM][FP], Frag<T> (&r2nxt)[RCKM][FP]) {
     const int y = y0 + it * TR;
-    const int s_it = (base + it * TR) % R;
+    const int s_it = (base + it * TRr) % R;
 #ifdef SDDM_STAMPS
     const int dbg = a.dbg;
 #else
@@ -328,36 +346,71 @@
     for (int i = 0; i < FP; ++i)
 #pragma unroll
       for (int j = 0; j < FC; ++j) acc[i][j] = f32x4{0.f, 0.f, 0.f, 0.f};
-    const char* bptr[FP][3];
-#pragma unroll
-    for (int fp = 0; fp < FP; ++fp)
-#pragma unroll
-      for (int dy = 0; dy < 3; ++dy) {
-        int sl = s_it + prow[fp] + dy;
+    f32x4 tv[UPT];
+    if constexpr (PH) {
+      const char* bptr[2];
+#pragma unroll
+      for (int ta = 0; ta < 2; ++ta) {
+        int sl = s_it + srow + py + ta;
         sl = sl >= R ? sl - R : sl;
-        bptr[fp][dy] = ring + (sl * SLOT + (g * UPL * PL + pcol[fp] * 16));
-      }
-    f32x4 tv[UPT];
-#pragma unroll
-    for (int ck = 0; ck < NCK; ++ck) {
-#pragma unroll
-      for (int tap = 0; tap < 9; ++tap) {
-        const int dy = tap / 3, dx = tap - 3 * dy;
-        Frag<T> bf[FP];
-#pragma unroll
-        for (int fp = 0; fp < FP; ++fp)
-          bf[fp] = load_planes<T>((SDDM_ABL_STRIP & 256) ? bptr[fp][0] : bptr[fp][dy] + ck * 4 * UPL * PL + dx * 16, PL);
-#pragma unroll
-        for (int fc = 0; fc < FC; ++fc) {
-          const Frag<T> af = WREG ? wreg[WREG ? tap : 0][fc]
-                                  : load_planes<T>(abase + ((SDDM_ABL_STRIP & 16) ? 0 : (ck * 9 + tap) * 4 * UPL * WPL) + fc * 256, WPL);
+        bptr[ta] = ring + (sl * SLOT + (g * UPL * PL + scol * 16));
+      }
+      const char* aw = abase + py * (NTW * 4 * UPL * WPL);
+#pragma unroll
+      for (int ck = 0; ck < NCK; ++ck) {
+#pragma unroll
+        for (int ta = 0; ta < 2; ++ta) {
+          Frag<T> bf[3];
+#pragma unroll
+          for (int cx = 0; cx < 3; ++cx) bf[cx] = load_planes<T>(bptr[ta] + ck * 4 * UPL * PL + cx * 16, PL);
+#pragma unroll
+          for (int px = 0; px < 2; ++px)
+#pragma unroll
+            for (int tb = 0; tb < 2; ++tb) {
+              const int tw = px * 4 + ta * 2 + tb;
+#pragma unroll
+              for (int fc = 0; fc < FC; ++fc) {
+                const Frag<T> af = WREG ? wreg[WREG ? tw : 0][fc]
+                                        : load_planes<T>(aw + (ck * NTAP + tw) * 4 * UPL * WPL + fc * 256, WPL);
+                if (!(dbg & 8)) mfma_frag(acc[px][fc], af, bf[px + tb]);
+              }
+            }
+#pragma unroll
+          for (int k = 0; k < UPT; ++k)
+            if (decltype(LX)::value && ck * 2 + ta == k * 2 * NCK / UPT) tv[k] = (dbg & 2) ? fill[k] : xform_unit(fill, it + 1, k);
+        }
+      }
+    } else {
+      const char* bptr[FP][3];
+#pragma unroll
+      for (int fp = 0; fp < FP; ++fp)
+#pragma unroll
+        for (int dy = 0; dy < 3; ++dy) {
+          int sl = s_it + prow[fp] + dy;
+          sl = sl >= R ? sl - R : sl;
+          bptr[fp][dy] = ring + (sl * SLOT + (g * UPL * PL + pcol[fp] * 16));
+        }
+#pragma unroll
+      for (int ck = 0; ck < NCK; ++ck) {
+#pragma unroll
+        for (int tap = 0; tap < 9; ++tap) {
+          const int dy = tap / 3, dx = tap - 3 * dy;
+          Frag<T> bf[FP];
 #pragma unroll
           for (int fp = 0; fp < FP; ++fp)
-            if (!(dbg & 8)) mfma_frag(acc[fp][fc], af, bf[fp]);
+            bf[fp] = load_planes<T>((SDDM_ABL_STRIP & 256) ? bptr[fp][0] : bptr[fp][dy] + ck * 4 * UPL * PL + dx * 16, PL);
+#pragma unroll
+          for (int fc = 0; fc < FC; ++fc) {
+            const Frag<T> af = WREG ? wreg[WREG ? tap : 0][fc]
+                                    : load_planes<T>(abase + ((SDDM_ABL_STRIP & 16) ? 0 : (ck * 9 + tap) * 4 * UPL * WPL) + fc * 256, WPL);
+#pragma unroll
+            for (int fp = 0; fp < FP; ++fp)
+              if (!(dbg & 8)) mfma_frag(acc[fp][fc], af, bf[fp]);
+          }
+#pragma unroll
+          for (int k = 0; k < UPT; ++k)
+            if (decltype(LX)::value && ck * 9 + tap == k * 9 * NCK / UPT) tv[k] = (dbg & 2) ? fill[k] : xform_unit(fill, it + 1, k);
         }
-#pragma unroll
-        for (int k = 0; k < UPT; ++k)
-          if (decltype(LX)::value && ck * 9 + tap == k * 9 * NCK / UPT) tv[k] = (dbg & 2) ? fill[k] : xform_unit(fill, it + 1, k);
       }
     }
     if constexpr (RES == 2) {
@@ -401,9 +454,10 @@
   asm volatile("s_waitcnt vmcnt(%0) lgkmcnt(0)\n\ts_barrier" :: "n"(NYOUNG) : "memory");
   if constexpr (WREG) {
 #pragma unroll
-    for (int tap = 0; tap < 9; ++tap)
-#pragma unroll
-      for (int fc = 0; fc < FC; ++fc) wreg[tap][fc] = load_planes<T>(abase + tap * 4 * UPL * WPL + fc * 256, WPL);
+    for (int tap = 0; tap < NTW; ++tap)
+#pragma unroll
+      for (int fc = 0; fc < FC; ++fc)
+        wreg[tap][fc] = load_planes<T>(abase + ((PH ? py * NTW : 0) + tap) * 4 * UPL * WPL + fc * 256, WPL);
   }
   SDDM_STAMP(a, 3);
   using yes = std::integral_constant<bool, true>;
@@ -444,19 +498,19 @@
   SDDM_STAMP(a, 7);
 }
 
-template <typename T, int FC, int W, int CIN, int MPI>
+template <typename T, int FC, int W, int CIN, int MPI, bool PH = false>
 static size_t strip_lds(const ConvArgs& a) {
-  constexpr int ES = (int)sizeof(T), NBLK = 16 * FC, TR = MPI / W, R = 2 * TR + 2;
-  constexpr int UPP = CIN * ES / 16, PL = ((W + 2) * 16 + 255) / 256 * 256;
-  size_t n = (size_t)R * UPP * PL + (size_t)(CIN / 32) * 9 * 4 * (ES / 2) * NBLK * 16;
+  constexpr int ES = (int)sizeof(T), NBLK = 16 * FC, TR = MPI / W, R = 2 * (PH ? TR / 2 : TR) + 2;
+  constexpr int UPP = CIN * ES / 16, PL = (((PH ? W / 2 : W) + 2) * 16 + 255) / 256 * 256;
+  size_t n = (size_t)R * UPP * PL + (size_t)(CIN / 32) * (PH ? 16 : 9) * 4 * (ES / 2) * NBLK * 16;
   if (a.res_mode == 2) n += (size_t)((a.RCA + a.RCB) * ES / 16) * NBLK * 16;
   n += (size_t)2 * CIN * 4 + (size_t)(MPI / 32) * NBLK * 3 * 4;
   return n;
 }
 
-template <typename T, int FC, int W, int CIN, int MPI, int SH = 0>
+template <typename T, int FC, int W, int CIN, int MPI, int SH = 0, bool PH = false>
 static hipError_t strip_go(const ConvArgs& a, int SR, int B, hipStream_t s, size_t* lo) {
-  const size_t lds = strip_lds<T, FC, W, CIN, MPI>(a);
+  const size_t lds = strip_lds<T, FC, W, CIN, MPI, PH>(a);
   if (lo) { *lo = lds; return hipSuccess; }
   constexpr int TR = MPI / W;
   if (lds > kLdsBytes || a.Ho % SR || SR % (2 * TR) || a.Cout % (16 * FC) || a.res_mode < 0 || a.res_mode > 2 ||
@@ -466,7 +520,10 @@
   if (sizeof(T) == 2 && (!a.wgt_t || (a.res_mode == 2 && !a.res_wgt_t))) return hipErrorInvalidValue;
   const dim3 grid = xcd_grid(a.Ho / SR, B, a.Cout / (16 * FC)), blk(MPI * 2);
   if (a.res_mode != 0 && !a.gamma) return hipErrorInvalidValue;
-  if constexpr (SH > 0) {
+  if constexpr (PH) {
+    if (a.res_mode != 0 || a.gamma || a.upsample != 2 || a.Hi * 2 != a.Ho || a.Wi * 2 != a.Wo) return hipErrorInvalidValue;
+    hipLaunchKernelGGL((conv_strip_kernel<T, FC, W, CIN, MPI, 0, false, SH, true>), grid, blk, lds, s, a, SR);
+  } else if constexpr (SH > 0) {
     constexpr ConvShape c = kStripShapes[SH];
     hipLaunchKernelGGL((conv_strip_kernel<T, FC, W, CIN, MPI, c.res, c.gn != 0, SH>), grid, blk, lds, s, a, SR);
   } else if (a.res_mode == 0 && !a.gamma) hipLaunchKernelGGL((conv_strip_kernel<T, FC, W, CIN, MPI, 0, false, 0>), grid, blk, lds, s, a, SR);
@@ -474,6 +531,19 @@
   else if (a.res_mode == 1) hipLaunchKernelGGL((conv_strip_kernel<T, FC, W, CIN, MPI, 1, true, 0>), grid, blk, lds, s, a, SR);
   else hipLaunchKernelGGL((conv_strip_kernel<T, FC, W, CIN, MPI, 2, true, 0>), grid, blk, lds, s, a, SR);
   return hipGetLastError();
+}
+
+template <typename T, int FC, int W, int CIN, int MPI, int SH = 0>
+static hipError_t strip_go_up(const ConvArgs& a, int SR, int B, hipStream_t s, size_t* lo) {
+  if (a.upsample == 2) {
+    if constexpr ((MPI / W) % 2 == 0) {
+      return strip_go<T, FC, W, CIN, MPI, SH, true>(a, SR, B, s, lo);
+    } else {
+      if (lo) *lo = (size_t)1 << 40;
+      return hipErrorInvalidValue;
+    }
+  }
+  return strip_go<T, FC, W, CIN, MPI, SH, false>(a, SR, B, s, lo);
 }
 
 template <typename T, int SH>
@@ -485,7 +555,8 @@
   } else {
     constexpr ConvShape c = kStripShapes[SH];
     if (strip_shape_matches(c, nblk, mpi, SR, a)) {
-      e = strip_go<T, c.cfg / 16, c.Wo, c.CA + c.CB, c.nw, SH>(a, SR, B, s, nullptr);
+      if constexpr (c.up != 0) e = strip_go_up<T, c.cfg / 16, c.Wo, c.CA + c.CB, c.nw, SH>(a, SR, B, s, nullptr);
+      else e = strip_go<T, c.cfg / 16, c.Wo, c.CA + c.CB, c.nw, SH>(a, SR, B, s, nullptr);
       return true;
     }
     return strip_shape_go<T, SH + 1>(a, nblk, mpi, SR, B, s, e);
@@ -500,7 +571,7 @@
   const int Cin = a.CA + a.CB;
 #define SDDM_STRIP(FCV, WV, CV)                                                                   \
   if (nblk == 16 * FCV && a.Wo == WV && Cin == CV)                                                \
-    return mpi == 256 ? strip_go<T, FCV, WV, CV, 256>(a, SR, B, s, lo) : strip_go<T, FCV, WV, CV, 128>(a, SR, B, s, lo);
+    return mpi == 256 ? strip_go_up<T, FCV, WV, CV, 256>(a, SR, B, s, lo) : strip_go_up<T, FCV, WV, CV, 128>(a, SR, B, s, lo);
   SDDM_STRIP(2, 128, 32) SDDM_STRIP(2, 128, 64) SDDM_STRIP(4, 128, 32) SDDM_STRIP(4, 128, 64)
   SDDM_STRIP(2, 64, 32) SDDM_STRIP(2, 64, 64) SDDM_STRIP(2, 64, 128)
   SDDM_STRIP(4, 64, 32) SDDM_STRIP(4, 64, 64) SDDM_STRIP(4, 64, 128)
diff --git a/speech-denoising-diffusion-model-2_amd/csrc/sddm_runtime.cpp b/speech-denoising-diffusion-model-2_amd/csrc/sddm_runtime.cpp
--- a/speech-denoising-diffusion-model-2_amd/csrc/sddm_runtime.cpp
+++ b/speech-denoising-diffusion-model-2_amd/csrc/sddm_runtime.cpp
@@ -23,6 +23,7 @@
 int compute_schedule(const std::string& schedule, int T, double linear_start, double linear_end,
                      float* out);
 }
+#include "upsample_phase.h"
 using namespace sddm;
 
 static thread_local std::string g_last_error;
@@ -344,6 +345,37 @@
       blobs.push_back(std::move(bt));
     }
   };
+  auto add_conv3_phase = [&](const std::string& name, const Param& w) {
+    const int co = (int)w.shape[0], ci = (int)w.shape[1];
+    const int cop = (co + 63) / 64 * 64, nch = ci / 32;
+    std::vector<float> ph((size_t)16 * co * ci);
+    upsample_phase_weights(w.data.data(), co, ci, ph.data());
+    Blob b, bf, bt;
+    b.bytes.assign((size_t)cop * ci * 16 * es, 0);
+    bf.bytes.assign((size_t)co * ci * 16 * es, 0);
+    if (dt != DT_F32) bt.bytes.assign((size_t)co * ci * 16 * es, 0);
+    for (int t = 0; t < 16; ++t)
+      for (int o = 0; o < co; ++o)
+        for (int i = 0; i < ci; ++i) {
+          const float v = ph[((size_t)t * co + o) * ci + i];
+          store_elem(b.bytes.data(), (((size_t)o * nch + i / 32) * 16 + t) * 32 + (i % 32), v, dt);
+          const int s = (i / 32) * 16 + t, l = (o % 16) + 16 * ((i % 32) / 8);
+          store_elem(bf.bytes.data(), (((size_t)(o / 16) * (nch * 16) + s) * 64 + l) * 8 + i % 8, v, dt);
+          if (dt != DT_F32)
+            store_elem(bt.bytes.data(), ((((size_t)(i / 32) * 16 + t) * 4 + (i % 32) / 8) * co + o) * 8 + i % 8, v, dt);
+        }
+    b.off = A.reserve(b.bytes.size());
+    c->woff[name + "_p"] = b.off;
+    blobs.push_back(std::move(b));
+    bf.off = A.reserve(bf.bytes.size());
+    c->woff[name + "_pf"] = bf.off;
+    blobs.push_back(std::move(bf));
+    if (dt != DT_F32) {
+      bt.off = A.reserve(bt.bytes.size());
+      c->woff[name + "_pt"] = bt.off;
+      blobs.push_back(std::move(bt));
+    }
+  };
   auto add_conv1 = [&](const std::string& name, const Param& w) {
     const int co = (int)w.shape[0], ci = (int)w.shape[1];
     const int cop = (co + 63) / 64 * 64;
@@ -410,6 +442,7 @@
       sc += L.cout;
     } else if (L.kind == 2 || L.kind == 3) {
       add_conv3(n + ".w", P(n + ".conv.weight"));
+      if (L.kind == 3) add_conv3_phase(n + ".w", P(n + ".conv.weight"));
       add_f32(n + ".b", P(n + ".conv.bias").data);
     } else {
       add_f32(n + ".gamma", P(n + ".block.0.weight").data);
@@ -558,7 +591,7 @@
   return true;
 }
 
-static bool choose_conv(int dt, int B, int Cin, int RC, int res_mode, int Ho, int Wo, int Cout, bool s2, bool up,
+static bool choose_conv(int dt, int B, int Cin, int RC, int res_mode, int Ho, int Wo, int Cout, bool s2, int up,
                         ConvChoice& ch, int want_mt = 0, int want_nw = 0, int kind = 0, int ka = 0, int want_nb = 0) {
   ConvArgs a{};
   a.CA = Cin; a.CB = 0; a.RCA = RC; a.RCB = 0; a.res_mode = res_mode; a.Ho = Ho; a.Wo = Wo; a.Cout = Cout;
@@ -576,9 +609,12 @@
       if (env_mpi && mpi != env_mpi) continue;
       const int TRs = mpi / Wo;
       if (Ho % TRs) continue;
+      if (up == 2 && (TRs & 1)) continue;
       for (int ni = 0; ni < 2; ++ni) {
         const int nb = nbs[ni];
-        if (conv_strip_lds_bytes(dt, nb, mpi, a) > kLdsBytes) continue;
+        ConvArgs as = a;
+        as.upsample = up;
+        if (conv_strip_lds_bytes(dt, nb, mpi, as) > kLdsBytes) continue;
         const int nz = (Cout + nb - 1) / nb;
         int SR = 0;
         const int target = env_blocks ? env_blocks : 256;
@@ -649,7 +685,9 @@
   if (!tuned && dt == DT_F16)
     for (const auto& tt : c->tunes)
       if (tt.B == PB && tt.N == N && tt.dtype == DT_BF16) { tuned = &tt; break; }
-  auto pick = [&](const std::string& name, int Cin, int RC, int res_mode, int Ho, int Wo, int cout, bool s2, bool up,
+  const char* up_env = std::getenv("SDDM_UP_PHASE");
+  const bool up_phase = up_env ? std::atoi(up_env) != 0 : dt != DT_F32;
+  auto pick = [&](const std::string& name, int Cin, int RC, int res_mode, int Ho, int Wo, int cout, bool s2, int up,
                   ConvChoice& ch) {
     int wm = 0, wn = 0, wb = 0, kind = 0, ka = 0;
     if (tuned) {
@@ -676,8 +714,8 @@
   auto res_block = [&](const std::string& n, int xa, int xb, int cin, int cout) -> int {
     const int H = tres[xa].H, Wd = tres[xa].W;
     ConvChoice c1, c2;
-    if (!pick(n + ".block1", cin, 0, 0, H, Wd, cout, false, false, c1)) return -1;
-    if (!pick(n + ".block2", cout, cin, cin != cout ? 2 : 1, H, Wd, cout, false, false, c2)) return -1;
+    if (!pick(n + ".block1", cin, 0, 0, H, Wd, cout, false, 0, c1)) return -1;
+    if (!pick(n + ".block2", cout, cin, cin != cout ? 2 : 1, H, Wd, cout, false, 0, c2)) return -1;
     const int g1 = new_gn(xa, xb, n + ".block1");
     const int h = new_tensor(cout, H, Wd, c1.n_tiles, c1.TR * c1.TW);
     { Step st; st.type = ST_CONV; st.w = n + ".block1"; st.rb = n; st.srcA = xa; st.srcB = xb; st.gn = g1;
@@ -700,7 +738,7 @@
       if (tres[cur].H % 2 || tres[cur].W % 2) FAIL(SDDM_ERR_SHAPE, "odd size before %s", L.name.c_str());
       const int H = tres[cur].H / 2, Wd = tres[cur].W / 2;
       ConvChoice ch;
-      if (!pick(L.name, tres[cur].C, 0, 0, H, Wd, L.cout, true, false, ch)) FAIL(SDDM_ERR_SHAPE, "no tile for %s", L.name.c_str());
+      if (!pick(L.name, tres[cur].C, 0, 0, H, Wd, L.cout, true, 0, ch)) FAIL(SDDM_ERR_SHAPE, "no tile for %s", L.name.c_str());
       const int o = new_tensor(L.cout, H, Wd, ch.n_tiles, ch.TR * ch.TW);
       Step st; st.type = ST_CONV; st.w = L.name; st.srcA = cur; st.out = o; st.s2 = 1; st.cout = L.cout; st.ch = ch;
       prog.push_back(st);
@@ -724,9 +762,10 @@
     } else {
       const int H = tres[cur].H * 2, Wd = tres[cur].W * 2;
       ConvChoice ch;
-      if (!pick(L.name, tres[cur].C, 0, 0, H, Wd, L.cout, false, true, ch)) FAIL(SDDM_ERR_SHAPE, "no tile for %s", L.name.c_str());
+      if (!pick(L.name, tres[cur].C, 0, 0, H, Wd, L.cout, false, up_phase ? 2 : 1, ch)) FAIL(SDDM_ERR_SHAPE, "no tile for %s", L.name.c_str());
       const int o = new_tensor(L.cout, H, Wd, ch.n_tiles, ch.TR * ch.TW);
-      Step st; st.type = ST_CONV; st.w = L.name; st.srcA = cur; st.out = o; st.up = 1; st.cout = L.cout; st.ch = ch;
+      Step st; st.type = ST_CONV; st.w = L.name; st.srcA = cur; st.out = o; st.cout = L.cout; st.ch = ch;
+      st.up = (up_phase && ch.strip) ? 2 : 1;
       prog.push_back(st);
       cur = o;
     }
@@ -765,6 +804,11 @@
     a.wgt = WV(st.w + ".w"); a.bias = WF(st.w + ".b");
     a.wgt_t = c->woff.count(st.w + ".w_t") ? WV(st.w + ".w_t") : nullptr;
     a.wgt_f = WV(st.w + ".w_f");
+    if (st.up == 2) {
+      a.wgt = WV(st.w + ".w_p");
+      a.wgt_t = c->woff.count(st.w + ".w_pt") ? WV(st.w + ".w_pt") : nullptr;
+      a.wgt_f = WV(st.w + ".w_pf");
+    }
     a.res_mode = st.res_mode;
     const int Cin = a.CA + a.CB;
     bytes = (double)B * a.Hi * a.Wi * Cin * es + (double)B * a.Ho * a.Wo * a.Cout * es +
diff --git a/speech-denoising-diffusion-model-2_amd/csrc/upsample_phase.cpp b/speech-denoising-diffusion-model-2_amd/csrc/upsample_phase.cpp
--- /dev/null
+++ b/speech-denoising-diffusion-model-2_amd/csrc/upsample_phase.cpp
@@ -0,0 +1,33 @@
+#pragma clang fp contract(off)
+#include "sddm_hip.h"
+#include "upsample_phase.h"
+
+namespace sddm {
+
+void upsample_phase_weights(const float* w, int cout, int cin, float* out16) {
+  for (int t = 0; t < 16; ++t) {
+    const int py = t >> 3, px = (t >> 2) & 1, a = (t >> 1) & 1, b = t & 1;
+    const int ky0 = (py == 0) ? (a == 0 ? 0 : 1) : (a == 0 ? 0 : 2), ky1 = (py == 0) ? (a == 0 ? 1 : 3) : (a == 0 ? 2 : 3);
+    const int kx0 = (px == 0) ? (b == 0 ? 0 : 1) : (b == 0 ? 0 : 2), kx1 = (px == 0) ? (b == 0 ? 1 : 3) : (b == 0 ? 2 : 3);
+    for (int o = 0; o < cout; ++o)
+      for (int i = 0; i < cin; ++i) {
+        const float* k = w + ((size_t)o * cin + i) * 9;
+        float s = 0.f;
+        bool first = true;
+        for (int ky = ky0; ky < ky1; ++ky)
+          for (int kx = kx0; kx < kx1; ++kx) {
+            s = first ? k[ky * 3 + kx] : s + k[ky * 3 + kx];
+            first = false;
+          }
+        out16[((size_t)t * cout + o) * cin + i] = s;
+      }
+  }
+}
+
+}
+
+extern "C" int sddm_upsample_phase_weights(const float* w, int cout, int cin, float* out16) {
+  if (!w || !out16 || cout <= 0 || cin <= 0) return SDDM_ERR_INVALID_ARG;
+  sddm::upsample_phase_weights(w, cout, cin, out16);
+  return SDDM_OK;
+}
diff --git a/speech-denoising-diffusion-model-2_amd/csrc/upsample_phase.h b/speech-denoising-diffusion-model-2_amd/csrc/upsample_phase.h
--- /dev/null
+++ b/speech-denoising-diffusion-model-2_amd/csrc/upsample_phase.h
@@ -0,0 +1,8 @@
+#pragma once
+#include <stddef.h>
+
+namespace sddm {
+
+void upsample_phase_weights(const float* w, int cout, int cin, float* out16);
+
+}
diff --git a/speech-denoising-diffusion-model-2_amd/sddm_hip/__init__.py b/speech-denoising-diffusion-model-2_amd/sddm_hip/__init__.py
--- a/speech-denoising-diffusion-model-2_amd/sddm_hip/__init__.py
+++ b/speech-denoising-diffusion-model-2_amd/sddm_hip/__init__.py
@@ -21,7 +21,7 @@
            "sddm_load_param", "sddm_missing_params", "sddm_sample", "sddm_sample_noise", "sddm_sample_continuous",
            "sddm_network_forward",
            "sddm_transition", "sddm_q_sample", "sddm_log_spectrogram", "sddm_set_conv_tuning", "sddm_initial_state", "sddm_schedule", "sddm_profile_enable",
-           "sddm_profile_read", "sddm_profile_ops")
+           "sddm_profile_read", "sddm_profile_ops", "sddm_upsample_phase_weights")
 
 _lib = None
 
@@ -57,6 +57,7 @@
                                         ctypes.POINTER(i64), ctypes.POINTER(ctypes.c_double),
                                         ctypes.POINTER(ctypes.c_double)]
         L.sddm_profile_ops.argtypes = [vp, ctypes.c_char_p, i64]
+        L.sddm_upsample_phase_weights.argtypes = [vp, c_int, c_int, vp]
         for name in EXPORTS:
             if name not in ("sddm_last_error", "sddm_destroy", "sddm_abi_version"):
                 getattr(L, name).restype = c_int
@@ -88,6 +89,15 @@
     return dict(zip(TABLE_NAMES, out))
 
 
+def upsample_phase_weights(w):
+    w = np.ascontiguousarray(w, dtype=np.float32)
+    cout, cin = w.shape[:2]
+    assert w.shape == (cout, cin, 3, 3)
+    out = np.empty((2, 2, 2, 2, cout, cin), dtype=np.float32)
+    check(lib().sddm_upsample_phase_weights(w.ctypes.data, cout, cin, out.ctypes.data))
+    return out
+
+
 def _ptr(t):
     return ctypes.c_void_p(0 if t is None else t.data_ptr())
 
diff --git a/speech-denoising-diffusion-model-2_amd/sddm_hip/build.py b/speech-denoising-diffusion-model-2_amd/sddm_hip/build.py
--- a/speech-denoising-diffusion-model-2_amd/sddm_hip/build.py
+++ b/speech-denoising-diffusion-model-2_amd/sddm_hip/build.py
@@ -17,7 +17,7 @@
     BUILD = os.path.join(HERE, "_build")
     LIB = os.path.join(HERE, "libsddm_hip.so")
 SOURCES = ["kernels.hip", "conv_strip.hip", "conv_strip_bf16.hip", "conv_strip_f16.hip", "conv_strip_f32.hip", "conv_deep.hip", "conv_tile.hip", "conv_chain.hip", "diffwave.hip", "wavegrad.hip", "waveunet.hip", "q_sample.hip", "stft.hip", "sddm_runtime.cpp",
-           "schedule.cpp"]
+           "schedule.cpp", "upsample_phase.cpp"]
 HIPCC = os.environ.get("HIPCC", "/opt/rocm/bin/hipcc")
 ARCH = os.environ.get("SDDM_OFFLOAD_ARCH", "gfx950")
 FLAGS = ["-O3", "-std=c++17", "-fPIC", f"--offload-arch={ARCH}", "-I", CSRC, "-I", INCLUDE,
```

New measurement: 25.81 audio_s/s, median of 3. No clear change (+0.1%).
